# e-sha/dvs_of_training_framework

Hardware: AMD Instinct MI355X
Metric: training samples/sec (256x256x5 event voxels) (higher is better)
Workload: dtype f32; 1 GPU; EV_FlowNet 256x256x5-bin synthetic events, batch 8 per GPU, fp32 (BASELINE.json configs[1]); full step: voxelise + fwd + multi-scale loss + bwd + AdamW-amsgrad; global_batch=8, parallelism=dp1

## Files before the change

dvs_of_training_framework_amd/conv.py:

```python
import ctypes

import torch

from . import _lib

_vp = ctypes.c_void_p
_C = _lib.CONSTANTS

ACT_NONE, ACT_RELU, ACT_MISH = _C['DVSOF_ACT_NONE'], _C['DVSOF_ACT_RELU'], _C['DVSOF_ACT_MISH']
NHWC, NCHW = _C['DVSOF_NHWC'], _C['DVSOF_NCHW']
WGRAD_SKIP_FLAT = _C['DVSOF_CONV_WGRAD_SKIP_FLAT']

Src = _lib.STRUCTS['dvsof_src_t']
ConvDesc = _lib.STRUCTS['dvsof_conv_desc_t']
GradDst = _lib.STRUCTS['dvsof_grad_dst_t']

MFMA_F32, MFMA_BF16, MFMA_BF16X3, MFMA_BF16_TWINS = 0, 1, 2, 3


def twin(t):
    return torch.empty(t.shape, dtype=torch.bfloat16, device=t.device)


def to_bf16(src):
    dst = torch.empty(src.numel(), dtype=torch.bfloat16, device=src.device)
    _lib.check(_lib.lib().dvsof_to_bf16(src.data_ptr(), dst.data_ptr(),
                                         src.numel(), _lib.stream()),
               'dvsof_to_bf16')
    return dst


def to_bf16_many(tensors):
    tensors = list(tensors)
    out = [torch.empty(t.numel(), dtype=torch.bfloat16, device=t.device)
           for t in tensors]
    for i in range(0, len(tensors), 16):
        chunk, dst = tensors[i:i + 16], out[i:i + 16]
        n = len(chunk)
        src_p = (_vp * n)(*[t.data_ptr() for t in chunk])
        dst_p = (_vp * n)(*[t.data_ptr() for t in dst])
        sizes = (ctypes.c_size_t * n)(*[t.numel() for t in chunk])
        _lib.check(_lib.lib().dvsof_to_bf16_many(src_p, dst_p, sizes, n,
                                                  _lib.stream()),
                   'dvsof_to_bf16_many')
    return out


UP_NONE, UP_NEAREST, UP_ZERO = 0, 1, 2

_KERNELS = sorted((v, k[len('DVSOF_KERNEL_'):]) for k, v in _C.items() if k.startswith('DVSOF_KERNEL_'))
assert [v for v, _ in _KERNELS] == list(range(len(_KERNELS)))
globals().update(('K_' + name, v) for v, name in _KERNELS)
KERNEL_NAMES = tuple(name.lower() for _, name in _KERNELS)


def last_kernel(kind):
    v = _lib.lib().dvsof_conv2d_last_kernel(kind)
    return v & 255, v >> 8


def make_desc(srcs, B, H, W, Cout, ksize=3, stride=1, pad=1, upsample=False,
              act=ACT_NONE, mfma=MFMA_F32):
    d = ConvDesc()
    d.nsrc = len(srcs)
    for i, src in enumerate(srcs):
        t, C, layout = src[:3]
        d.src[i].p = t.data_ptr()
        d.src[i].C = C
        d.src[i].layout = layout
        d.src[i].p16 = _lib.ptr(src[3]) if len(src) > 3 else None
    d.B, d.H, d.W = B, H, W
    if upsample is True or upsample is False:
        upsample = UP_NEAREST if upsample else UP_NONE
    assert upsample in (UP_NONE, UP_NEAREST, UP_ZERO)
    d.upsample = upsample
    d.ksize, d.stride, d.pad = ksize, stride, pad
    d.Cout, d.act, d.mfma = Cout, act, mfma
    return d


def out_size(desc):
    up = 2 if desc.upsample else 1
    ho = (desc.H * up + 2 * desc.pad - desc.ksize) // desc.stride + 1
    wo = (desc.W * up + 2 * desc.pad - desc.ksize) // desc.stride + 1
    return ho, wo


_PLAN = {}


def _plan(desc):
    key = (desc.nsrc, tuple((desc.src[i].C, desc.src[i].layout)
                            for i in range(desc.nsrc)), desc.B, desc.H, desc.W,
           desc.upsample, desc.ksize, desc.stride, desc.pad, desc.Cout,
           desc.mfma)
    p = _PLAN.get(key)
    if p is None:
        lib, ref = _lib.lib(), ctypes.byref(desc)
        raw = desc.Cout * desc.ksize ** 2 * sum(desc.src[i].C
                                                for i in range(desc.nsrc))
        p = _PLAN[key] = (raw, lib.dvsof_conv2d_fwd_weight_elems(ref),
                          lib.dvsof_conv2d_dgrad_weight_elems(ref),
                          lib.dvsof_conv2d_scratch_bytes(ref),
                          lib.dvsof_conv2d_wgrad_workspace_bytes(ref))
    return p


def _scratch(desc, device):
    n = _plan(desc)[3]
    if n == 0:
        desc.scratch, desc.scratch_bytes = None, 0
        return None
    t = torch.empty(n // 4, dtype=torch.float32, device=device)
    desc.scratch, desc.scratch_bytes = t.data_ptr(), n
    return t


def winograd_chain(desc, kind):
    return bool(_lib.lib().dvsof_conv2d_winograd_chain(ctypes.byref(desc), kind))


def winograd_tile(desc, kind):
    return _lib.lib().dvsof_conv2d_winograd_tile(ctypes.byref(desc), kind)


def winograd_form(desc, channels, device):
    tiles = desc.B * (desc.H // 4) * (desc.W // 4)
    return torch.empty(36 * tiles * channels, dtype=torch.float32, device=device)


def _chain(desc, pre=None, nxt=None, nxt_gout=None, gout=None):
    desc.winograd_pre = _lib.ptr(pre)
    desc.winograd_next = _lib.ptr(nxt)
    desc.winograd_next_gout = _lib.ptr(nxt_gout)
    desc.winograd_gout = _lib.ptr(gout)


def conv_fwd(desc, weight, bias, device, residual=None, want_z=False,
             keep_input_transform=False, weight16=None, bias_cls=None,
             wino_pre=None, wino_next=None):
    ho, wo = out_size(desc)
    y = torch.empty(desc.B, ho, wo, desc.Cout, dtype=torch.float32,
                    device=device)
    z = torch.empty_like(y) if want_z else None
    desc._y16 = twin(y) if desc.mfma == MFMA_BF16_TWINS else None
    desc.y16 = _lib.ptr(desc._y16)
    desc.w16 = _lib.ptr(weight16)
    desc.bias_cls = _lib.ptr(bias_cls)
    ws = _scratch(desc, device)
    _chain(desc, pre=wino_pre, nxt=wino_next)
    _lib.check(_lib.lib().dvsof_conv2d_fwd(
        ctypes.byref(desc), weight.data_ptr(), _lib.ptr(bias),
        _lib.ptr(residual), y.data_ptr(), _lib.ptr(z), _lib.stream()),
        'dvsof_conv2d_fwd')
    _chain(desc)
    desc._wino_input = (wino_pre if wino_pre is not None else ws) \
        if keep_input_transform else None
    return y, z


def prepare(desc, weight, want_dgrad, phase_weights=None, want16=False):
    lib = _lib.lib()
    raw, nf, ndg, nscratch, _ = _plan(desc)
    dg_only = phase_weights is not None
    if dg_only:
        w_fwd = phase_weights
    else:
        w_fwd = weight if nf == raw else torch.empty(
            nf, dtype=torch.float32, device=weight.device)
    w_dg = torch.empty(ndg, dtype=torch.float32, device=weight.device) \
        if want_dgrad else None
    make_fwd = not dg_only and nf != raw
    w_fwd16 = w_dg16 = None
    if make_fwd or want_dgrad:
        wino = nscratch > 0
        wp = weight.data_ptr()
        fp = w_fwd.data_ptr() if (nf != raw) else None
        if dg_only:
            fp = None
        if want16 and not wino:
            dev = weight.device
            if make_fwd or (nf == raw and want_dgrad and not dg_only):
                w_fwd16 = torch.empty(nf, dtype=torch.bfloat16, device=dev)
            if want_dgrad:
                w_dg16 = torch.empty(ndg, dtype=torch.bfloat16, device=dev)
            _lib.check(lib.dvsof_conv2d_prepare16(
                ctypes.byref(desc), wp, fp, _lib.ptr(w_dg), _lib.ptr(w_fwd16),
                _lib.ptr(w_dg16), _lib.stream()), 'dvsof_conv2d_prepare16')
        else:
            _lib.check(lib.dvsof_conv2d_prepare(
                ctypes.byref(desc), wp, fp, _lib.ptr(w_dg), _lib.stream()),
                'dvsof_conv2d_prepare')
            if want16:
                w_fwd16 = to_bf16(w_fwd) if make_fwd else None
                w_dg16 = to_bf16(w_dg) if w_dg is not None else None
    if want16:
        return w_fwd, w_dg, w_fwd16, w_dg16
    return w_fwd, w_dg


def flip_transpose(weight, Cout, ksize, Ctot):
    wt = torch.empty(Ctot * ksize * ksize * Cout, dtype=torch.float32,
                     device=weight.device)
    _lib.check(_lib.lib().dvsof_weight_flip_transpose(
        weight.data_ptr(), wt.data_ptr(), Cout, ksize, Ctot, _lib.stream()),
        'dvsof_weight_flip_transpose')
    return wt


def conv_dgrad(desc, weight_t, gout, dsts, bwd_act=ACT_NONE, weight16=None,
               gout16=None, wino_pre=None, wino_next=None, wino_next_gout=None):
    arr = (GradDst * len(dsts))()
    for i, d in enumerate(dsts):
        arr[i].p = d['p'].data_ptr()
        arr[i].addend = _lib.ptr(d.get('addend'))
        arr[i].addend2 = _lib.ptr(d.get('addend2'))
        arr[i].actsrc = _lib.ptr(d.get('actsrc'))
        arr[i].p16 = _lib.ptr(d.get('p16'))
        arr[i].head_w = _lib.ptr(d.get('head_w'))
        arr[i].head_gflow = _lib.ptr(d.get('head_gflow'))
        arr[i].head_x = _lib.ptr(d.get('head_x'))
        arr[i].head_part = _lib.ptr(d.get('head_part'))
    desc.w16 = _lib.ptr(weight16)
    desc.gout16 = _lib.ptr(gout16)
    ws = _scratch(desc, gout.device)
    _chain(desc, pre=wino_pre, nxt=wino_next, nxt_gout=wino_next_gout)
    _lib.check(_lib.lib().dvsof_conv2d_dgrad(
        ctypes.byref(desc), weight_t.data_ptr(), gout.data_ptr(), arr,
        bwd_act, _lib.stream()), 'dvsof_conv2d_dgrad')
    _chain(desc)


def flow_fold_weights(w, Cout, Ctot, cx_off, Cx, cf_off, wh):
    out = torch.empty(Cout * 9 * (Ctot - 2), dtype=torch.float32, device=w.device)
    _lib.check(_lib.lib().dvsof_flow_fold_weights(
        w.data_ptr(), Cout, Ctot, cx_off, Cx, cf_off, wh.data_ptr(),
        out.data_ptr(), _lib.stream()), 'dvsof_flow_fold_weights')
    return out


def flow_fold_bias(w, Cout, Ctot, cf_off, bh, bias):
    be = torch.empty(Cout, dtype=torch.float32, device=w.device)
    bc = torch.empty(9 * Cout, dtype=torch.float32, device=w.device)
    _lib.check(_lib.lib().dvsof_flow_fold_bias(
        w.data_ptr(), Cout, Ctot, cf_off, bh.data_ptr(), _lib.ptr(bias),
        be.data_ptr(), bc.data_ptr(), _lib.stream()), 'dvsof_flow_fold_bias')
    return be, bc


def flow_fold_grads(dW, w, Cout, Ctot, cx_off, Cx, cf_off, wh, bh, db_conv, g,
                    B, H, W, dwh, dbh):
    n = _lib.lib().dvsof_flow_fold_workspace_bytes(B, Cout)
    ws = torch.empty(n // 4 + 1, dtype=torch.float32, device=g.device)
    _lib.check(_lib.lib().dvsof_flow_fold_grads(
        dW.data_ptr(), w.data_ptr(), Cout, Ctot, cx_off, Cx, cf_off,
        wh.data_ptr(), bh.data_ptr(), db_conv.data_ptr(), g.data_ptr(), B, H,
        W, dwh.data_ptr(), dbh.data_ptr(), ws.data_ptr(), ws.numel() * 4,
        _lib.stream()), 'dvsof_flow_fold_grads')


def conv_wgrad(desc, gout, dweight, dbias, gout16=None, skip_flat=False,
               wino_gout=None):
    desc.gout16 = _lib.ptr(gout16)
    desc.flags = WGRAD_SKIP_FLAT if skip_flat else 0
    nbytes = _plan(desc)[4]
    ws = torch.empty(max(nbytes // 4, 4), dtype=torch.float32,
                     device=gout.device)
    kept = getattr(desc, '_wino_input', None)
    desc.winograd_input = kept.data_ptr() if kept is not None else None
    _chain(desc, gout=wino_gout)
    _lib.check(_lib.lib().dvsof_conv2d_wgrad(
        ctypes.byref(desc), gout.data_ptr(), dweight.data_ptr(),
        _lib.ptr(dbias), ws.data_ptr(), ws.numel() * 4, _lib.stream()),
        'dvsof_conv2d_wgrad')
    _chain(desc)


def first_dgrad(gz, weight, B, C, H, W):
    _lib.require_cuda(gz, weight)
    assert gz.dtype == torch.float32 and gz.is_contiguous()
    assert gz.numel() == B * (H // 2) * (W // 2) * 64
    assert tuple(weight.shape) == (64, C, 3, 3) and \
        weight.permute(0, 2, 3, 1).is_contiguous(), \
        'enc.0 weight: channels_last [64,C,3,3]'
    out = torch.empty(B, C, H, W, dtype=torch.float32, device=gz.device)
    _lib.check(_lib.lib().dvsof_first_dgrad(
        gz.data_ptr(), weight.data_ptr(), B, C, H, W, out.data_ptr(),
        _lib.stream()), 'dvsof_first_dgrad')
    return out


def head_fwd(x, w, bias, B, H, W, C):
    flow = torch.empty(B, 2, H, W, dtype=torch.float32, device=x.device)
    _lib.check(_lib.lib().dvsof_flow_head_fwd(
        x.data_ptr(), w.data_ptr(), _lib.ptr(bias), flow.data_ptr(), B, H, W,
        C, _lib.stream()), 'dvsof_flow_head_fwd')
    return flow


def heads_fwd(items, B, out=None):
    n = len(items)
    flows = out if out is not None else [
        torch.empty(B, 2, H, W, dtype=torch.float32, device=x.device)
        for x, _, _, H, W, _ in items]
    arr = lambda ts: (_vp * n)(*[_lib.ptr(t) for t in ts])
    ints = lambda k: (ctypes.c_int * n)(*[it[k] for it in items])
    _lib.check(_lib.lib().dvsof_flow_heads_fwd(
        n, arr([it[0] for it in items]), arr([it[1] for it in items]),
        arr([it[2] for it in items]), arr(flows), B, ints(3), ints(4), ints(5),
        _lib.stream()), 'dvsof_flow_heads_fwd')
    return flows


def dgrad_fuses_head(desc):
    return bool(_lib.lib().dvsof_conv2d_dgrad_fuses_head(ctypes.byref(desc)))


def dgrad_head_rows(desc):
    return _lib.lib().dvsof_conv2d_dgrad_head_rows(ctypes.byref(desc))


def dgrad_head_part(desc, C, device):
    rows = _lib.lib().dvsof_conv2d_dgrad_head_rows(ctypes.byref(desc))
    if rows <= 0:
        return None
    return torch.empty(rows, 2 * C + 2, dtype=torch.float32, device=device)


def head_reduce(part, C, dw, dbias):
    _lib.check(_lib.lib().dvsof_flow_head_reduce(
        part.data_ptr(), part.shape[0], C, dw.data_ptr(), _lib.ptr(dbias),
        _lib.stream()), 'dvsof_flow_head_reduce')


def head_bwd(x, w, gflow, gx_in, actsrc, act, gx, dw, dbias, B, H, W, C,
             gx16=None):
    nbytes = _lib.lib().dvsof_flow_head_bwd_workspace_bytes(B, H, W, C)
    ws = torch.empty(nbytes // 4, dtype=torch.float32, device=x.device)
    _lib.check(_lib.lib().dvsof_flow_head_bwd(
        x.data_ptr(), w.data_ptr(), gflow.data_ptr(), _lib.ptr(gx_in),
        _lib.ptr(actsrc), act, _lib.ptr(gx), dw.data_ptr(),
        _lib.ptr(dbias), B, H, W, C, ws.data_ptr(), nbytes, _lib.ptr(gx16),
        _lib.stream()), 'dvsof_flow_head_bwd')


def act_bwd(dy, actsrc, act, out=None):
    out = dy if out is None else out
    _lib.check(_lib.lib().dvsof_act_bwd(
        dy.data_ptr(), actsrc.data_ptr(), act, out.data_ptr(), dy.numel(),
        _lib.stream()), 'dvsof_act_bwd')
    return out
```

dvs_of_training_framework_amd/csrc/conv_api.hip:

```cpp
#include "conv_host.h"

static thread_local int t_last_kernel[3] = {0, 0, 0};
static thread_local int t_kind = 0;
void conv_note_kernel(int family, int mode) { t_last_kernel[t_kind] = family | mode << 8; }
static void conv_begin(int kind)
{
    t_kind = kind;
    t_last_kernel[kind] = DVSOF_KERNEL_NONE;
}
static int conv_retag(int rc, int family)
{
    if (rc == DVSOF_OK && t_last_kernel[t_kind]) conv_note_kernel(family, t_last_kernel[t_kind] >> 8);
    return rc;
}

namespace {

GSrc make_src(const float *p, int C, int layout, int H, int W, const void *p16 = nullptr)
{
    GSrc s;
    s.p = p;
    s.p16 = layout == DVSOF_NHWC ? (const unsigned short *)p16 : nullptr;
    s.C = C;
    if (layout == DVSOF_NCHW) {
        s.sb = (long long)C * H * W;
        s.sy = W;
        s.sx = 1;
        s.sc = H * W;
        s.flat = 1;
    } else {
        s.sb = (long long)H * W * C;
        s.sy = W * C;
        s.sx = C;
        s.sc = 1;
        s.flat = ((C & 3) || C < BK) ? 1 : 0;
    }
    return s;
}

bool desc_ok(const dvsof_conv_desc_t *d, int &Ctot, int &Ho, int &Wo)
{
    if (!d || d->nsrc < 1 || d->nsrc > 3 || d->B < 1 || d->H < 1 || d->W < 1) return false;
    if (d->ksize != 1 && d->ksize != 3 && d->ksize != 5) return false;
    if (d->stride != 1 && d->stride != 2) return false;
    if (d->upsample < 0 || d->upsample > 2) return false;
    if (d->upsample && d->stride != 1) return false;
    if (d->upsample == 2 &&
        !(d->ksize == 3 && d->pad == 1 && d->nsrc == 1 && d->src[0].layout == DVSOF_NHWC &&
          d->src[0].C % BK == 0 && d->mfma != 3))
        return false;
    if (d->Cout < 1 || d->pad < 0 || d->pad >= d->ksize) return false;
    Ctot = 0;
    for (int i = 0; i < d->nsrc; ++i) {
        if (!d->src[i].p || d->src[i].C < 1) return false;
        Ctot += d->src[i].C;
    }
    const int up = d->upsample ? 2 : 1;
    Ho = (d->H * up + 2 * d->pad - d->ksize) / d->stride + 1;
    Wo = (d->W * up + 2 * d->pad - d->ksize) / d->stride + 1;
    if (Ho < 1 || Wo < 1) return false;
    if ((long long)d->B * Ho * Wo > 0x7fffffffLL) return false;
    if ((long long)d->B * d->H * up * d->W * up > 0x7fffffffLL) return false;
    return true;
}

int operand_mode(const dvsof_conv_desc_t *d) { return (d->mfma >= 1 && d->mfma <= 3) ? d->mfma : 0; }

template <class Params>
void layer_geometry(Params &P, const dvsof_conv_desc_t *d, const ConvClass &c)
{
    const int up = d->upsample ? 2 : 1;
    P.B = d->B;
    P.Hv = d->H * up;
    P.Wv = d->W * up;
    P.up = d->upsample ? UP_NEAREST : UP_NONE;
    P.Ho = c.Ho;
    P.Wo = c.Wo;
    P.stride = d->stride;
    P.pad = d->pad;
    P.ks = d->ksize;
    P.M = d->B * c.Ho * c.Wo;
}

template <class Params>
void four_phases(Params &P, int h, int w, int pad, int ph_pad)
{
    P.up = UP_NONE;
    P.Hv = P.Ho = h;
    P.Wv = P.Wo = w;
    P.ks = 2;
    P.stride = 1;
    P.pad = pad;
    P.M = P.B * h * w;
    P.nph = 4;
    P.ph_pad = ph_pad;
}
void phase_strides(int &sy, int &sx, int &ph_y, int &ph_x)
{
    ph_y = sy;
    ph_x = sx;
    sy *= 2;
    sx *= 2;
}

void fill_wgrad(const dvsof_conv_desc_t *d, const ConvClass &c, WGradParams &P)
{
    P.mfma_bf16 = d->mfma == 3 ? 1 : operand_mode(d);
    P.nsrc = d->nsrc;
    for (int i = 0; i < d->nsrc; ++i)
        P.src[i] = make_src(d->src[i].p, d->src[i].C, d->src[i].layout, d->H, d->W,
                            d->mfma == 3 ? d->src[i].p16 : nullptr);
    P.gout16 = d->mfma == 3 ? (const unsigned short *)d->gout16 : nullptr;
    P.twins = P.gout16 != nullptr && (d->Cout % 8) == 0;
    for (int i = 0; i < d->nsrc; ++i)
        if (!P.src[i].flat && (!P.src[i].p16 || (P.src[i].C % 8))) P.twins = 0;
    layer_geometry(P, d, c);
    P.Cout = d->Cout;
    P.Cin_tot = c.Ctot;
    P.nph = 1;
    P.S = 1;
    P.g_sb = (long long)c.Ho * c.Wo * d->Cout;
    P.g_sy = c.Wo * d->Cout;
    P.g_sx = d->Cout;
    if (c.wgrad == WG_SUBPIXEL) {
        four_phases(P, d->H, d->W, d->pad, 1);
        phase_strides(P.g_sy, P.g_sx, P.g_py, P.g_px);
    }
}

int fill_flat(const dvsof_conv_desc_t *d, const ConvClass &c, const float *gout, FlatWG *F)
{
    int n = 0, coff = 0;
    for (int i = 0; i < d->nsrc; ++i) {
        const GSrc g = make_src(d->src[i].p, d->src[i].C, d->src[i].layout, d->H, d->W);
        if (g.flat) {
            FlatWG &f = F[n++];
            f.S = g;
            f.gout = gout;
            layer_geometry(f, d, c);
            f.Cout = d->Cout;
            f.ncol = d->ksize * d->ksize * g.C;
            f.coff = coff;
            f.Cin_tot = c.Ctot;
        }
        coff += d->src[i].C;
    }
    return n;
}

__global__ __launch_bounds__(256) void channel_sum_partial_kernel(const float *__restrict__ g,
                                                                  long long npix, int C,
                                                                  float *__restrict__ part)
{
    const int per = 256 / C, c = threadIdx.x % C, r = threadIdx.x / C;
    float a = 0.f;
    if (r < per)
        for (long long p = (long long)blockIdx.x * per + r; p < npix; p += (long long)gridDim.x * per)
            a += g[p * C + c];
    __shared__ float sm[256];
    sm[threadIdx.x] = a;
    __syncthreads();
    if (threadIdx.x < C) {
        float t = 0.f;
        for (int j = 0; j < per; ++j) t += sm[j * C + threadIdx.x];
        part[(size_t)blockIdx.x * C + threadIdx.x] = t;
    }
}
__global__ __launch_bounds__(256) void channel_sum_final_kernel(const float *__restrict__ part,
                                                                int nblocks, int C,
                                                                float *__restrict__ out)
{
    const int c = blockIdx.x * 4 + (threadIdx.x >> 6), lane = threadIdx.x & 63;
    if (c >= C) return;
    double a = 0;
    for (int b = lane; b < nblocks; b += 64) a += (double)part[(size_t)b * C + c];
    a = wave_sum(a);
    if (lane == 0) out[c] = (float)a;
}

}

ConvClass conv_classify(const dvsof_conv_desc_t *d)
{
    ConvClass c = {};
    c.ok = desc_ok(d, c.Ctot, c.Ho, c.Wo);
    if (!c.ok) return c;
    const bool subpixel = d->upsample == 1 && d->ksize == 3 && d->pad == 1 && d->stride == 1;
    const bool transposed = d->upsample == 2;
    const bool phased2 = !d->upsample && d->stride == 2 && d->ksize == 3 && d->pad == 1 &&
                         (d->H % 2 == 0) && (d->W % 2 == 0);
    const bool first = first_layer_shape(d->nsrc, d->src[0].layout == DVSOF_NCHW, d->src[0].C, d->Cout, d->H,
                                         d->W, d->ksize, d->stride, d->pad, d->upsample) && !d->bias_cls;
    const bool wino = d->nsrc == 1 &&
                      wino_eligible_shape(d->nsrc, d->src[0].layout == DVSOF_NHWC, d->src[0].C, d->Cout, d->B,
                                          d->H, d->W, d->ksize, d->stride, d->pad, d->upsample, d->mfma);
    c.wino_mode = d->mfma == 2 ? 2 : 0;
    const int wg_tile = wino ? wino_wgrad_tile(d->B, d->H, d->W, c.wino_mode) : 0;
    bool min9 = false, min9_dgrad = false;
    if (subpixel) {
        int C[3] = {0, 0, 0}, nhwc[3] = {0, 0, 0};
        for (int i = 0; i < d->nsrc; ++i) {
            C[i] = d->src[i].C;
            nhwc[i] = d->src[i].layout == DVSOF_NHWC;
        }
        min9 = min9_shape_ok(d->mfma, d->nsrc, C, nhwc, d->Cout, d->H, d->W);
        min9_dgrad = min9 && min9_dgrad_shape_ok(C, d->Cout, d->H);
    }
    c.fwd = first ? FWD_FIRST : wino ? FWD_WINO : min9 ? FWD_MIN9 : subpixel ? FWD_SUBPIXEL
          : transposed ? FWD_TRANSPOSED : FWD_GENERAL;
    c.dgrad = min9_dgrad ? DG_MIN9 : wino ? DG_WINO : subpixel ? DG_SUBPIXEL : phased2 ? DG_PHASED2
            : transposed ? DG_TRANSPOSED : d->upsample ? DG_QUAD : d->stride == 2 ? DG_ZERO2 : DG_PLAIN;
    c.wgrad = transposed ? WG_TRANSPOSED : wg_tile ? WG_WINO : first ? WG_FIRST : subpixel ? WG_SUBPIXEL
            : WG_GENERAL;
    if (wino) {
        c.wino_tile[0] = c.wino_tile[1] = wino_tile(d->B, d->H, d->W, c.wino_mode);
        c.wino_tile[2] = wg_tile;
        c.wino_chain[0] = wino_chain_ok(d->B, d->H, d->W, d->Cout, c.wino_mode);
        c.wino_chain[1] = wino_chain_ok(d->B, d->H, d->W, c.Ctot, c.wino_mode);
    }
    c.head_folds = min9_dgrad || (subpixel && d->src[0].layout == DVSOF_NHWC);
    return c;
}

extern "C" {

int dvsof_conv2d_fwd(const dvsof_conv_desc_t *d, const float *weight, const float *bias,
                     const float *residual, float *y, float *z, void *stream)
{
    conv_begin(0);
    const ConvClass c = conv_classify(d);
    if (!c.ok || !weight || !y) return DVSOF_EINVAL;
    hipStream_t st = as_stream(stream);
    unsigned short *y16 = d->mfma == 3 ? (unsigned short *)d->y16 : nullptr;
    if (c.fwd == FWD_FIRST && !residual)
        return first_fwd_launch(d->src[0].p, d->B, c.Ctot, d->H, d->W, weight, bias, d->act, y, z, y16, st);
    if (d->winograd_next_gout || (c.fwd != FWD_WINO && (d->winograd_pre || d->winograd_next)))
        return DVSOF_EINVAL;
    const int Cout = d->Cout;
    GConvParams P = {};
    P.nsrc = d->nsrc;
    for (int i = 0; i < d->nsrc; ++i)
        P.src[i] = make_src(d->src[i].p, d->src[i].C, d->src[i].layout, d->H, d->W, d->src[i].p16);
    P.ndst = 1;
    P.dst[0] = {y, residual, nullptr, nullptr, (long long)c.Ho * c.Wo * Cout, c.Wo * Cout, Cout, 1, Cout, 0, 0, y16};
    P.W = weight;
    P.W16 = d->mfma == 3 ? (const unsigned short *)d->w16 : nullptr;
    P.bias = bias;
    P.bias_cls = d->bias_cls;
    P.out_H = c.Ho;
    P.out_W = c.Wo;
    P.zout = z;
    layer_geometry(P, d, c);
    P.N = Cout;
    P.Cin_tot = c.Ctot;
    P.act = d->act;
    P.mfma_bf16 = operand_mode(d);
    P.bwd_act = ACT_NONE;
    P.nph = 1;
    switch (c.fwd) {
    case FWD_WINO: {
        const WinoChain ch = {d->winograd_pre, d->winograd_next, nullptr};
        return wino_launch(P, (float *)d->scratch, d->scratch_bytes / sizeof(float), ch, st);
    }
    case FWD_MIN9:
    case FWD_SUBPIXEL:
        four_phases(P, d->H, d->W, d->pad, 1);
        break;
    case FWD_TRANSPOSED:
        four_phases(P, d->H, d->W, 0, 0);
        P.ph_exact = 1;
        break;
    default: break;
    }
    if (P.nph == 4) {
        P.w_phase_stride = (long long)Cout * 4 * c.Ctot;
        phase_strides(P.dst[0].sy, P.dst[0].sx, P.dst[0].ph_y, P.dst[0].ph_x);
    }
    if (c.fwd == FWD_MIN9) return fwd_min_launch(P, st);
    if (c.fwd == FWD_SUBPIXEL && fwd_patch_eligible(P))
        return fwd_patch_launch(P, st);
    const int rc = gconv_launch(P, 0, st);
    return c.fwd == FWD_TRANSPOSED ? conv_retag(rc, DVSOF_KERNEL_TRANSPOSED) : rc;
}

int dvsof_conv2d_dgrad_fuses_head(const dvsof_conv_desc_t *d)
{
    const ConvClass c = conv_classify(d);
    return c.ok && c.head_folds ? 1 : 0;
}

int dvsof_conv2d_dgrad_head_rows(const dvsof_conv_desc_t *d)
{
    const ConvClass c = conv_classify(d);
    if (!c.ok || c.dgrad != DG_MIN9) return 0;
    return d->B * (d->H / 8) * (d->W / 16);
}

int dvsof_conv2d_dgrad(const dvsof_conv_desc_t *d, const float *weight_t, const float *gout,
                       const dvsof_grad_dst_t *dst, int bwd_act, void *stream)
{
    conv_begin(1);
    const ConvClass c = conv_classify(d);
    if (!c.ok || !weight_t || !gout || !dst) return DVSOF_EINVAL;
    hipStream_t st = as_stream(stream);
    GConvParams P = {};
    P.nsrc = 1;
    P.src[0] = make_src(gout, d->Cout, DVSOF_NHWC, c.Ho, c.Wo, d->mfma == 3 ? d->gout16 : nullptr);
    P.ndst = d->nsrc;
    for (int i = 0; i < d->nsrc; ++i) {
        if (!dst[i].p) return DVSOF_EINVAL;
        const GSrc g = make_src(nullptr, d->src[i].C, d->src[i].layout, d->H, d->W);
        P.dst[i] = {dst[i].p, dst[i].addend, dst[i].addend2, dst[i].actsrc, g.sb, g.sy, g.sx, g.sc, g.C, 0, 0,
                    (d->mfma == 3 && d->src[i].layout == DVSOF_NHWC) ? (unsigned short *)dst[i].p16 : nullptr,
                    dst[i].head_w, dst[i].head_gflow, dst[i].head_x, dst[i].head_part};
        if ((dst[i].head_w != nullptr) != (dst[i].head_gflow != nullptr)) return DVSOF_EINVAL;
        if ((dst[i].head_x != nullptr) != (dst[i].head_part != nullptr)) return DVSOF_EINVAL;
        if (dst[i].head_part && (!dst[i].head_w || i != 0)) return DVSOF_EINVAL;
        if (dst[i].head_w && (i != 0 || !c.head_folds)) return DVSOF_EINVAL;
        if (dst[i].head_part && c.dgrad != DG_MIN9) return DVSOF_EINVAL;
    }
    P.W = weight_t;
    P.W16 = d->mfma == 3 ? (const unsigned short *)d->w16 : nullptr;
    P.B = d->B;
    P.N = c.Ctot;
    P.Cin_tot = d->Cout;
    P.act = ACT_NONE;
    P.mfma_bf16 = operand_mode(d);
    P.bwd_act = bwd_act;
    P.nph = 1;
    P.up = UP_NONE;
    P.Hv = c.Ho;
    P.Wv = c.Wo;
    P.Ho = d->H;
    P.Wo = d->W;
    P.ks = d->ksize;
    P.stride = 1;
    P.pad = d->ksize - 1 - d->pad;
    switch (c.dgrad) {
    case DG_MIN9:
    case DG_SUBPIXEL:
        P.ks = 4;
        P.stride = 2;
        P.pad = 1;
        break;
    case DG_PHASED2:
        four_phases(P, d->H / 2, d->W / 2, 0, 0);
        P.ph_exact = 1;
        P.w_phase_stride = (long long)c.Ctot * 4 * d->Cout;
        for (int i = 0; i < d->nsrc; ++i) phase_strides(P.dst[i].sy, P.dst[i].sx, P.dst[i].ph_y, P.dst[i].ph_x);
        break;
    case DG_TRANSPOSED:
        P.stride = 2;
        P.pad = 1;
        break;
    case DG_QUAD:
        P.Ho = 2 * d->H;
        P.Wo = 2 * d->W;
        P.quad = 1;
        break;
    case DG_ZERO2:
        P.up = UP_ZERO;
        P.Hv = 2 * c.Ho;
        P.Wv = 2 * c.Wo;
        break;
    default: break;
    }
    P.M = d->B * P.Ho * P.Wo;
    if (c.dgrad == DG_MIN9) return dgrad_min_launch(P, st);
    if (c.dgrad == DG_WINO) {
        const WinoChain ch = {d->winograd_pre, d->winograd_next, d->winograd_next_gout};
        return wino_launch(P, (float *)d->scratch, d->scratch_bytes / sizeof(float), ch, st);
    }
    if (d->winograd_pre || d->winograd_next || d->winograd_next_gout) return DVSOF_EINVAL;
    const int rc = gconv_launch(P, 0, st);
    return c.dgrad == DG_PHASED2 ? conv_retag(rc, DVSOF_KERNEL_STRIDE2_PHASED) : rc;
}

size_t dvsof_conv2d_scratch_bytes(const dvsof_conv_desc_t *d)
{
    const ConvClass c = conv_classify(d);
    if (!c.ok || c.fwd != FWD_WINO) return 0;
    return wino_scratch_floats(d->B, d->H, d->W, c.Ctot, d->Cout, c.wino_mode) * sizeof(float);
}

static dvsof_conv_desc_t adjoint_of_transposed(const dvsof_conv_desc_t *d, int Ctot, const float *gy)
{
    dvsof_conv_desc_t a = *d;
    a.nsrc = 1;
    a.src[0].p = gy;
    a.src[0].C = d->Cout;
    a.src[0].layout = DVSOF_NHWC;
    a.src[0].p16 = nullptr;
    a.H = 2 * d->H;
    a.W = 2 * d->W;
    a.upsample = 0;
    a.stride = 2;
    a.Cout = Ctot;
    a.scratch = nullptr;
    a.scratch_bytes = 0;
    a.winograd_input = nullptr;
    return a;
}
static int channel_sum_blocks(long long npix, int C)
{
    const long long per = 256 / C, want = (npix + per * 8 - 1) / (per * 8);
    return (int)(want < 1 ? 1 : want > 1024 ? 1024 : want);
}

size_t dvsof_conv2d_wgrad_workspace_bytes(const dvsof_conv_desc_t *d)
{
    const ConvClass c = conv_classify(d);
    if (!c.ok) return 0;
    switch (c.wgrad) {
    case WG_TRANSPOSED: {
        static const float dummy = 0.f;
        const dvsof_conv_desc_t a = adjoint_of_transposed(d, c.Ctot, &dummy);
        size_t n = dvsof_conv2d_wgrad_workspace_bytes(&a);
        n = (n + 255) & ~(size_t)255;
        n += (size_t)c.Ctot * 9 * d->Cout * sizeof(float);
        if (d->Cout <= 256)
            n += (size_t)channel_sum_blocks((long long)d->B * c.Ho * c.Wo, d->Cout) * d->Cout * sizeof(float);
        return n + 256;
    }
    case WG_WINO:
        return wino_wgrad_workspace_floats(d->B, d->H, d->W, c.Ctot, d->Cout, c.wino_mode) * sizeof(float) + 16;
    default: break;
    }
    WGradParams P = {};
    fill_wgrad(d, c, P);
    FlatWG F[3] = {};
    const int nflat = fill_flat(d, c, nullptr, F);
    size_t n = wgrad_plan(P, F, nflat, true, true).total;
    if (c.wgrad == WG_FIRST) {
        const size_t nf = first_wgrad_workspace_floats(d->B, c.Ctot, d->H, d->W);
        if (nf > n) n = nf;
    }
    return n * sizeof(float) + 16;
}

int dvsof_conv2d_wgrad(const dvsof_conv_desc_t *d, const float *gout, float *dweight, float *dbias,
                       void *ws, size_t ws_bytes, void *stream)
{
    conv_begin(2);
    const ConvClass c = conv_classify(d);
    if (!c.ok || !gout || !dweight) return DVSOF_EINVAL;
    hipStream_t st = as_stream(stream);
    const bool skip_flat = (d->flags & DVSOF_CONV_WGRAD_SKIP_FLAT) != 0;
    switch (c.wgrad) {
    case WG_TRANSPOSED: {
        if (dbias && d->Cout > 256) return DVSOF_EINVAL;
        const dvsof_conv_desc_t a = adjoint_of_transposed(d, c.Ctot, gout);
        size_t wsa = dvsof_conv2d_wgrad_workspace_bytes(&a);
        wsa = (wsa + 255) & ~(size_t)255;
        const size_t need = dvsof_conv2d_wgrad_workspace_bytes(d);
        if (!ws || ws_bytes < need) return DVSOF_ENOSPACE;
        float *dw_adj = (float *)((char *)ws + wsa);
        float *part = dw_adj + (size_t)c.Ctot * 9 * d->Cout;
        int rc = dvsof_conv2d_wgrad(&a, d->src[0].p, dw_adj, nullptr, ws, wsa, stream);
        if (rc) return rc;
        rc = dvsof_weight_flip_transpose(dw_adj, dweight, c.Ctot, 3, d->Cout, stream);
        if (rc) return rc;
        if (dbias) {
            const long long npix = (long long)d->B * c.Ho * c.Wo;
            const int nb = channel_sum_blocks(npix, d->Cout);
            hipLaunchKernelGGL(channel_sum_partial_kernel, dim3(nb), dim3(256), 0, st, gout, npix, d->Cout, part);
            DVSOF_LAUNCH_CHECK();
            hipLaunchKernelGGL(channel_sum_final_kernel, dim3((d->Cout + 3) / 4), dim3(256), 0, st,
                               (const float *)part, nb, d->Cout, dbias);
            DVSOF_LAUNCH_CHECK();
        }
        return DVSOF_OK;
    }
    case WG_WINO: {
        const float *v_in = c.wino_tile[0] == c.wino_tile[2] ? d->winograd_input : nullptr;
        const float *z_in = c.wino_tile[2] == 4 ? d->winograd_gout : nullptr;
        return wino_wgrad_launch(make_src(d->src[0].p, d->src[0].C, d->src[0].layout, d->H, d->W), v_in, z_in,
                                 gout, dweight, dbias, d->B, d->H, d->W, c.Ctot, d->Cout, c.wino_mode, (float *)ws,
                                 ws_bytes / sizeof(float), st);
    }
    case WG_FIRST:
        if (!skip_flat)
            return first_wgrad_launch(d->src[0].p, d->B, c.Ctot, d->H, d->W, gout, dweight, dbias, (float *)ws,
                                      ws_bytes / sizeof(float), st);
        break;
    default: break;
    }
    WGradParams P = {};
    fill_wgrad(d, c, P);
    P.gout = gout;
    FlatWG F[3] = {};
    const int nflat = skip_flat ? 0 : fill_flat(d, c, gout, F);
    return wgrad_launch(P, dweight, dbias, (float *)ws, ws_bytes / sizeof(float), F, nflat, st);
}

size_t dvsof_conv2d_fwd_weight_elems(const dvsof_conv_desc_t *d)
{
    const ConvClass c = conv_classify(d);
    if (!c.ok) return 0;
    const bool phases = c.fwd == FWD_MIN9 || c.fwd == FWD_SUBPIXEL || c.fwd == FWD_TRANSPOSED;
    return (size_t)d->Cout * c.Ctot * (c.fwd == FWD_WINO ? wino_components(d->B, d->H, d->W, c.wino_mode)
                                       : phases ? 16 : d->ksize * d->ksize);
}

size_t dvsof_conv2d_dgrad_weight_elems(const dvsof_conv_desc_t *d)
{
    const ConvClass c = conv_classify(d);
    if (!c.ok) return 0;
    const bool taps16 = c.dgrad == DG_MIN9 || c.dgrad == DG_SUBPIXEL || c.dgrad == DG_PHASED2;
    return (size_t)d->Cout * c.Ctot * (c.dgrad == DG_WINO ? wino_components(d->B, d->H, d->W, c.wino_mode)
                                       : taps16 ? 16 : d->ksize * d->ksize);
}

int dvsof_conv2d_winograd_tile(const dvsof_conv_desc_t *d, int kind)
{
    const ConvClass c = conv_classify(d);
    return c.ok ? c.wino_tile[kind == 2 ? 2 : 0] : 0;
}

int dvsof_conv2d_winograd_chain(const dvsof_conv_desc_t *d, int kind)
{
    const ConvClass c = conv_classify(d);
    return c.ok && (kind == 0 || kind == 1) && c.wino_chain[kind] ? 1 : 0;
}

int dvsof_conv2d_kernel_generation(const dvsof_conv_desc_t *d, int kind)
{
    const ConvClass c = conv_classify(d);
    if (!c.ok) return DVSOF_EINVAL;
    if (kind != 1 && c.fwd == FWD_FIRST) return 3;
    if (kind == 2) {
        for (int i = 0; i < d->nsrc; ++i) {
            const GSrc g = make_src(d->src[i].p, d->src[i].C, d->src[i].layout, d->H, d->W);
            if (!g.flat) return (c.Wo % BK == 0 && (!d->upsample || c.wgrad == WG_SUBPIXEL)) ? 2 : 1;
        }
        return 0;
    }
    if (kind == 1) return (d->Cout % BK == 0) ? 2 : 1;
    for (int i = 0; i < d->nsrc; ++i) {
        const GSrc g = make_src(d->src[i].p, d->src[i].C, d->src[i].layout, d->H, d->W);
        if (!g.flat) return (g.C % BK == 0) ? 2 : 1;
    }
    return 1;
}

int dvsof_conv2d_last_kernel(int kind)
{
    return (kind >= 0 && kind <= 2) ? t_last_kernel[kind] : 0;
}

int dvsof_conv2d_last_patch(int kind)
{
    switch (dvsof_conv2d_last_kernel(kind) & 255) {
    case DVSOF_KERNEL_FWD_MIN4:
    case DVSOF_KERNEL_FWD_MIN8:
    case DVSOF_KERNEL_DGRAD_MIN0:
    case DVSOF_KERNEL_DGRAD_MIN1:
    case DVSOF_KERNEL_DGRAD_MIN2:
    case DVSOF_KERNEL_WGRAD_MIN: return 2;
    case DVSOF_KERNEL_FWD_PATCH:
    case DVSOF_KERNEL_WGRAD_PATCH: return 1;
    default: return 0;
    }
}

int dvsof_conv2d_tile_id(const dvsof_conv_desc_t *d, int kind)
{
    const ConvClass c = conv_classify(d);
    if (!c.ok) return DVSOF_EINVAL;
    if (kind == 0) return gconv_pick_tile((long long)d->B * c.Ho * c.Wo, d->Cout);
    if (kind == 1) {
        const int up = (c.dgrad == DG_QUAD || c.dgrad == DG_TRANSPOSED) ? 2 : 1;
        int n = c.Ctot, trail = 0;
        for (int i = d->nsrc - 1; i > 0; --i) {
            const GSrc g = make_src(d->src[i].p, d->src[i].C, d->src[i].layout, d->H, d->W);
            if (!g.flat || trail + g.C > 4) break;
            trail += g.C;
        }
        if (up == 1 && c.dgrad != DG_PHASED2 && n - trail >= 32) n -= trail;
        return gconv_pick_tile((long long)d->B * d->H * up * d->W * up, n);
    }
    if (kind == 2) {
        WGradParams P = {};
        fill_wgrad(d, c, P);
        return wgrad_plan(P, nullptr, 0, false, true).tile;
    }
    return DVSOF_EINVAL;
}

}
```

dvs_of_training_framework_amd/csrc/conv_common.h:

```cpp
#pragma once
#include "common.h"

typedef float f32x16 __attribute__((ext_vector_type(16)));
typedef float f32x4 __attribute__((ext_vector_type(4)));
typedef float f32x4u __attribute__((ext_vector_type(4), aligned(4)));
typedef float f32x8 __attribute__((ext_vector_type(8)));
typedef __bf16 bf16x8 __attribute__((ext_vector_type(8)));

enum { UP_NONE = 0, UP_NEAREST = 1, UP_ZERO = 2 };
enum { ACT_NONE = 0, ACT_RELU = 1, ACT_MISH = 2 };

constexpr int CONV_NT = 256;
constexpr int BK = 16;
constexpr int LDK = BK + 4;

struct GSrc {
    const float *p;
    long long sb;
    int sy, sx, sc;
    int C;
    int flat;
    const unsigned short *p16;
};

struct GDst {
    float *p;
    const float *addend;
    const float *addend2;
    const float *actsrc;
    long long sb;
    int sy, sx, sc;
    int C;
    int ph_y, ph_x;
    unsigned short *p16;
    const float *head_w;
    const float *head_g;
    const float *head_x;
    float *head_part;
};

struct GConvParams {
    GSrc src[3];
    GDst dst[3];
    const float *W;
    const unsigned short *W16;
    const float *bias;
    const float *bias_cls;
    int out_H, out_W;
    float *zout;
    int nsrc, ndst;
    int B, Hv, Wv;
    int up;
    int Ho, Wo;
    int stride, pad, ks;
    int nph;
    int ph_pad;
    long long w_phase_stride;
    long long src_ph_stride;
    int N, Cin_tot, M;
    int quad;
    int act;
    int bwd_act;
    int mfma_bf16;
    int ph_exact;
    int xcd;
    int dbg;
};

struct WinoChain {
    const float *v_pre;
    float *v_next;
    float *z_next;
};

struct WGradParams {
    GSrc src[3];
    const float *gout;
    float *dW;
    float *dbias;
    int nsrc;
    int B, Hv, Wv, up, Ho, Wo, stride, pad, ks;
    int Cout, Cin_tot, M;
    int klen;
    int tile_begin[4];
    long long g_sb;
    int g_sy, g_sx;
    int g_py, g_px;
    int nph, ph_pad, S;
    int mfma_bf16;
    long long src_ph_stride;
    const unsigned short *gout16;
    int twins;
    int xcd;
};

struct FlatWG {
    GSrc S;
    const float *gout;
    int B, Hv, Wv, up, Ho, Wo, stride, pad, ks, Cout, M, ncol;
    int coff, Cin_tot;
};

__device__ __forceinline__ float mish_t(float x, float &n)
{
    n = __builtin_amdgcn_exp2f(fminf(x, 20.f) * 1.4426950408889634f);
    return n * (n + 2.f);
}

__device__ __forceinline__ unsigned short bf16_bits(float v)
{
    const __bf16 h = (__bf16)v;
    return __builtin_bit_cast(unsigned short, h);
}

__device__ __forceinline__ float act_fwd(float v, int act)
{
    if (act == ACT_RELU) return fmaxf(v, 0.f);
    if (act == ACT_MISH) {
        float n;
        const float t = mish_t(v, n);
        return v * (t * __builtin_amdgcn_rcpf(t + 2.f));
    }
    return v;
}

__device__ __forceinline__ float act_bwd(float s, int act)
{
    if (act == ACT_RELU) return s > 0.f ? 1.f : 0.f;
    if (act == ACT_MISH) {
        float n;
        const float t = mish_t(s, n);
        const float r = __builtin_amdgcn_rcpf(t + 2.f);
        const float th = t * r;
        const float sg = n * __builtin_amdgcn_rcpf(1.f + n);
        return th + (s > 20.f ? 20.f : s) * ((2.f * r) * (1.f + th)) * sg;
    }
    return 1.f;
}

template <int MODE, int TM, int TN>
__device__ __forceinline__ void mfma_k16(f32x16 (&acc)[TM][TN], const f32x4 (&a)[2][TM],
                                         const f32x4 (&b)[2][TN])
{
    if constexpr (MODE == 0) {
#pragma unroll
        for (int j = 0; j < 2; ++j)
#pragma unroll
            for (int i = 0; i < 4; ++i)
#pragma unroll
                for (int tm = 0; tm < TM; ++tm)
#pragma unroll
                    for (int tn = 0; tn < TN; ++tn)
                        acc[tm][tn] = __builtin_amdgcn_mfma_f32_32x32x2f32(a[j][tm][i], b[j][tn][i],
                                                                           acc[tm][tn], 0, 0, 0);
    } else {
        bf16x8 ah[TM], bh[TN], al[TM], bl[TN];
#pragma unroll
        for (int t = 0; t < TM; ++t) {
            const f32x8 v = __builtin_shufflevector(a[0][t], a[1][t], 0, 1, 2, 3, 4, 5, 6, 7);
            ah[t] = __builtin_convertvector(v, bf16x8);
            if constexpr (MODE == 2)
                al[t] = __builtin_convertvector(v - __builtin_convertvector(ah[t], f32x8), bf16x8);
        }
#pragma unroll
        for (int t = 0; t < TN; ++t) {
            const f32x8 v = __builtin_shufflevector(b[0][t], b[1][t], 0, 1, 2, 3, 4, 5, 6, 7);
            bh[t] = __builtin_convertvector(v, bf16x8);
            if constexpr (MODE == 2)
                bl[t] = __builtin_convertvector(v - __builtin_convertvector(bh[t], f32x8), bf16x8);
        }
#pragma unroll
        for (int tm = 0; tm < TM; ++tm)
#pragma unroll
            for (int tn = 0; tn < TN; ++tn) {
                if constexpr (MODE == 2) {
                    acc[tm][tn] = __builtin_amdgcn_mfma_f32_32x32x16_bf16(al[tm], bh[tn], acc[tm][tn], 0, 0, 0);
                    acc[tm][tn] = __builtin_amdgcn_mfma_f32_32x32x16_bf16(ah[tm], bl[tn], acc[tm][tn], 0, 0, 0);
                }
                acc[tm][tn] = __builtin_amdgcn_mfma_f32_32x32x16_bf16(ah[tm], bh[tn], acc[tm][tn], 0, 0, 0);
            }
    }
}

__device__ __forceinline__ void conv_row_offsets(const GConvParams &P, long long *rowO, int *rowC, int BM,
                                                 int r, bool valid, int b, int oy, int ox, int phy,
                                                 int phx)
{
    if (P.bias_cls) {
        const int Y = P.nph == 4 ? 2 * oy + phy : oy, X = P.nph == 4 ? 2 * ox + phx : ox;
        rowC[r] = valid ? 3 * (Y == 0 ? 1 : Y == P.out_H - 1 ? 2 : 0) + (X == 0 ? 1 : X == P.out_W - 1 ? 2 : 0)
                        : 0;
    }
    if (P.dst[0].head_w) rowC[r] = valid ? (b * 2 * P.Ho + oy) * P.Wo + ox : -1;
    if (P.quad) {
        oy >>= 1;
        ox >>= 1;
    }
    for (int d = 0; d < P.ndst; ++d) {
        const GDst &D = P.dst[d];
        rowO[d * BM + r] = valid ? (long long)b * D.sb + (long long)oy * D.sy + (long long)ox * D.sx +
                                       (long long)phy * D.ph_y + (long long)phx * D.ph_x
                                 : -1;
    }
}

template <int TM, int TN>
__device__ __forceinline__ void conv_epilogue(const GConvParams &P, f32x16 (&acc)[TM][TN],
                                              const long long *rowO, const int *rowC, int BM, int n0,
                                              int wr, int wc, int lane)
{
    const int lrow = lane & 31;
    bool has_add = false, has_add2 = false, has_as = false;
    for (int d = 0; d < P.ndst; ++d) {
        has_add |= P.dst[d].addend != nullptr;
        has_add2 |= P.dst[d].addend2 != nullptr;
        has_as |= P.dst[d].actsrc != nullptr;
    }
#pragma unroll
    for (int tn = 0; tn < TN; ++tn) {
        const int n = n0 + (wc * TN + tn) * 32 + lrow;
        const bool col_ok = n < P.N;
        int dsel = 0, off = 0, run = 0;
        float *dp = P.dst[0].p;
        unsigned short *dp16 = P.dst[0].p16;
        const float *a1 = P.dst[0].addend, *a2 = P.dst[0].addend2, *as = P.dst[0].actsrc;
        int sc = P.dst[0].sc;
        for (int d = 1; d < P.ndst; ++d) {
            run += P.dst[d - 1].C;
            if (n >= run) {
                dsel = d;
                off = run;
                dp = P.dst[d].p;
                dp16 = P.dst[d].p16;
                a1 = P.dst[d].addend;
                a2 = P.dst[d].addend2;
                as = P.dst[d].actsrc;
                sc = P.dst[d].sc;
            }
        }
        const long long *ro = rowO + dsel * BM;
        const long long cpart = (long long)(n - off) * sc;
        const float bias = (P.bias && col_ok) ? P.bias[n] : 0.f;
#ifdef DVSOF_NO_GENERAL_HEAD
        const bool has_head = false;
#else
        const bool has_head = P.dst[0].head_w != nullptr;
#endif
        float hw0 = 0.f, hw1 = 0.f;
        if (has_head && dsel == 0 && col_ok) {
            hw0 = P.dst[0].head_w[n];
            hw1 = P.dst[0].head_w[P.dst[0].C + n];
        }
#pragma unroll
        for (int tm = 0; tm < TM; ++tm) {
            const int rbase = (wr * TM + tm) * 32 + 4 * (lane >> 5);
            if (!P.quad) {
                long long o[16];
                float v[16];
#pragma unroll
                for (int reg = 0; reg < 16; ++reg) {
                    const long long r_ = ro[rbase + (reg & 3) + 8 * (reg >> 2)];
                    o[reg] = (col_ok && r_ >= 0) ? r_ + cpart : -1;
                    v[reg] = acc[tm][tn][reg] + bias;
                }
                if (P.bias_cls) {
#pragma unroll
                    for (int reg = 0; reg < 16; ++reg) {
                        const int c = rowC[rbase + (reg & 3) + 8 * (reg >> 2)];
                        if (c != 0 && col_ok) v[reg] += P.bias_cls[c * P.N + n];
                    }
                }
                if (has_add) {
                    float t[16];
#pragma unroll
                    for (int reg = 0; reg < 16; ++reg) t[reg] = (a1 && o[reg] >= 0) ? a1[o[reg]] : 0.f;
#pragma unroll
                    for (int reg = 0; reg < 16; ++reg) v[reg] = a1 ? v[reg] + t[reg] : v[reg];
                }
                if (has_add2) {
                    float t[16];
#pragma unroll
                    for (int reg = 0; reg < 16; ++reg) t[reg] = (a2 && o[reg] >= 0) ? a2[o[reg]] : 0.f;
#pragma unroll
                    for (int reg = 0; reg < 16; ++reg) v[reg] = a2 ? v[reg] + t[reg] : v[reg];
                }
                if (has_head) {
                    const long long hwp = (long long)P.Ho * P.Wo;
                    float g0[16], g1[16];
#pragma unroll
                    for (int reg = 0; reg < 16; ++reg) {
                        const int rg = rowC[rbase + (reg & 3) + 8 * (reg >> 2)];
                        g0[reg] = rg >= 0 ? P.dst[0].head_g[rg] : 0.f;
                        g1[reg] = rg >= 0 ? P.dst[0].head_g[rg + hwp] : 0.f;
                    }
#pragma unroll
                    for (int reg = 0; reg < 16; ++reg) v[reg] += g0[reg] * hw0 + g1[reg] * hw1;
                }
                if (has_as) {
                    float t[16];
#pragma unroll
                    for (int reg = 0; reg < 16; ++reg) t[reg] = (as && o[reg] >= 0) ? as[o[reg]] : 0.f;
#pragma unroll
                    for (int reg = 0; reg < 16; ++reg)
                        v[reg] = as ? v[reg] * act_bwd(t[reg], P.bwd_act) : v[reg];
                }
                if (P.zout) {
#pragma unroll
                    for (int reg = 0; reg < 16; ++reg)
                        if (o[reg] >= 0) P.zout[o[reg]] = v[reg];
                }
#pragma unroll
                for (int reg = 0; reg < 16; ++reg) v[reg] = act_fwd(v[reg], P.act);
#pragma unroll
                for (int reg = 0; reg < 16; ++reg)
                    if (o[reg] >= 0) dp[o[reg]] = v[reg];
                if (dp16) {
#pragma unroll
                    for (int reg = 0; reg < 16; ++reg)
                        if (o[reg] >= 0) dp16[o[reg]] = bf16_bits(v[reg]);
                }
            } else {
                long long o[4];
                float v[4];
#pragma unroll
                for (int g = 0; g < 4; ++g) {
                    const long long r_ = ro[rbase + 8 * g];
                    o[g] = (col_ok && r_ >= 0) ? r_ + cpart : -1;
                    v[g] = (acc[tm][tn][4 * g] + acc[tm][tn][4 * g + 1]) +
                           (acc[tm][tn][4 * g + 2] + acc[tm][tn][4 * g + 3]) + bias;
                }
                float t1[4], t2[4], t3[4];
#pragma unroll
                for (int g = 0; g < 4; ++g) {
                    t1[g] = (a1 && o[g] >= 0) ? a1[o[g]] : 0.f;
                    t2[g] = (a2 && o[g] >= 0) ? a2[o[g]] : 0.f;
                    t3[g] = (as && o[g] >= 0) ? as[o[g]] : 0.f;
                }
#pragma unroll
                for (int g = 0; g < 4; ++g) {
                    if (a1) v[g] += t1[g];
                    if (a2) v[g] += t2[g];
                    if (as) v[g] *= act_bwd(t3[g], P.bwd_act);
                    if (o[g] >= 0) dp[o[g]] = v[g];
                    if (dp16 && o[g] >= 0) dp16[o[g]] = bf16_bits(v[g]);
                }
            }
        }
    }
}
```

dvs_of_training_framework_amd/csrc/conv_host.h:

```cpp
#pragma once
#include "conv_common.h"

enum ConvFwdForm { FWD_GENERAL, FWD_FIRST, FWD_WINO, FWD_MIN9, FWD_SUBPIXEL, FWD_TRANSPOSED };
enum ConvDgradForm { DG_PLAIN, DG_MIN9, DG_WINO, DG_SUBPIXEL, DG_PHASED2, DG_TRANSPOSED, DG_QUAD, DG_ZERO2 };
enum ConvWgradForm { WG_GENERAL, WG_TRANSPOSED, WG_WINO, WG_FIRST, WG_SUBPIXEL };

struct ConvClass {
    bool ok;
    int Ctot, Ho, Wo;
    ConvFwdForm fwd;
    ConvDgradForm dgrad;
    ConvWgradForm wgrad;
    int wino_mode;
    int wino_tile[3];
    bool wino_chain[2];
    bool head_folds;
};
ConvClass conv_classify(const dvsof_conv_desc_t *d);

void conv_note_kernel(int family, int mode);

int gconv_launch(const GConvParams &P, int tile_hint, hipStream_t st);
int gconv_pick_tile(long long m, long long n);
bool gconv2_eligible(const GConvParams &P, long long max_src_bytes, long long w_bytes);
int gconv2_launch(const GConvParams &P, int tile, hipStream_t st);

enum WGVec { WGV_NONE, WGV_V1, WGV_V2, WGV_PATCH_TWINS, WGV_PATCH_F32, WGV_MIN9 };
enum WGFlat { WGF_NONE, WGF_V1, WGF_OWN };
enum WGBias { WGB_NONE, WGB_VECTOR, WGB_COLSUM, WGB_FLAT };
enum WGReduce { WGR_NONE, WGR_SLABS, WGR_SUBPIXEL, WGR_PATCH };
constexpr int WG_COLSUM_BLOCKS = 512;
constexpr int WG_FLAT_BLOCKS = 512;
constexpr int WG_MIN_CT = 64;
struct WGradPlan {
    int rc;
    WGVec vec;
    int tile, bn;
    int ntiles;
    int S, klen;
    WGFlat flat;
    bool flat_mfma[3];
    WGBias bias;
    bool bias_tail;
    WGReduce reduce;
    int zg;
    size_t bias_off, flat_off[3], total;
    int family, mode;
};
WGradPlan wgrad_plan(const WGradParams &P, const FlatWG *flat, int nflat, bool with_bias, bool sizing);
int wgrad_enumerate_tiles(WGradParams &P, int cols_per_channel, int width, bool vec, bool flat);
bool wgrad2_eligible(const WGradParams &P);
int wgrad_launch(WGradParams P, float *dW, float *dbias, float *ws, size_t ws_floats,
                 const FlatWG *flat, int nflat, hipStream_t st);
int wgrad2_launch(const WGradParams &P, int tile, int ntiles, hipStream_t st);
int wgrad_patch_launch(const WGradParams &P, bool f32, int ct, hipStream_t st);
int wgrad_min_launch(const WGradParams &P, hipStream_t st);
template <void (*KERNEL)(const WGradParams), int CT, int NT, int LDS>
int wgrad_resident_launch(const WGradParams &P0, hipStream_t st)
{
    WGradParams P = P0;
    const int nt = wgrad_enumerate_tiles(P, 1, CT, true, false);
    static bool attr_set = false;
    if (!attr_set) {
        DVSOF_HIP_TRY(hipFuncSetAttribute((const void *)KERNEL, hipFuncAttributeMaxDynamicSharedMemorySize, LDS));
        attr_set = true;
    }
    P.xcd = 1;
    hipLaunchKernelGGL(KERNEL, dim3(nt, P.Cout / 32, P.S), dim3(NT), LDS, st, P);
    DVSOF_LAUNCH_CHECK();
    return DVSOF_OK;
}

bool wino_eligible_shape(int nsrc, int layout_nhwc, int C, int N, int B, int H, int W, int ksize,
                         int stride, int pad, int upsample, int mfma);
int wino_tile(int B, int H, int W, int mfma);
int wino_components(int B, int H, int W, int mfma);
bool wino_chain_ok(int B, int H, int W, int N, int mfma);
size_t wino_scratch_floats(int B, int H, int W, int C, int N, int mfma);
int wino_prepare(const float *weight, float *U, float *Ut, int N, int C, int B, int H, int W, int mfma,
                 hipStream_t st);
int wino_launch(const GConvParams &P, float *scratch, size_t scratch_floats, const WinoChain &ch, hipStream_t st);
int wino_wgrad_tile(int B, int H, int W, int mfma);
size_t wino_wgrad_workspace_floats(int B, int H, int W, int C, int N, int mfma);
int wino_wgrad_launch(const GSrc &X, const float *V_in, const float *Z_in, const float *gout, float *dW, float *dbias, int B,
                      int H, int W, int C, int N, int mfma_bf16, float *ws, size_t ws_floats,
                      hipStream_t st);

bool first_layer_shape(int nsrc, int planar, int C, int Cout, int H, int W, int ksize, int stride,
                       int pad, int upsample);
int first_fwd_launch(const float *x, int B, int C, int H, int W, const float *w, const float *bias,
                     int act, float *y, float *z, unsigned short *y16, hipStream_t st);
size_t first_wgrad_workspace_floats(int B, int C, int H, int W);
int first_wgrad_launch(const float *x, int B, int C, int H, int W, const float *gout, float *dW,
                       float *dbias, float *ws, size_t ws_floats, hipStream_t st);

bool fwd_patch_eligible(const GConvParams &P);
int fwd_patch_launch(const GConvParams &P, hipStream_t st);
bool min9_shape_ok(int mfma, int nsrc, const int *C, const int *nhwc, int Cout, int H, int W);
int min9_prepare_fwd(const float *w, float *wt, int Cout, int Ctot, hipStream_t st);
int fwd_min_launch(const GConvParams &P, hipStream_t st);
bool min9_dgrad_shape_ok(const int *C, int Cout, int H);
int min9_prepare_dgrad(const float *w, float *wq, int Cout, int Ctot, hipStream_t st);
int dgrad_min_launch(const GConvParams &P, hipStream_t st);
```

dvs_of_training_framework_amd/csrc/dgrad_min.hip:

```cpp
#include "conv_host.h"
#include <stdlib.h>

namespace {

constexpr unsigned DM_OOB = 0x80000000u;
constexpr int DM_NT = 512;
constexpr int DM_NR = 8;
constexpr int DM_AARR = 9 * 1024 + 16;
constexpr int DM_AP = 4 * 9;
constexpr int DM_PR = 17;
constexpr int DM_NPAIR = (2 * DM_NR + 2) * DM_PR;
constexpr int DM_BPA = 5;
constexpr int DM_BARR = DM_BPA * 1024 + 16;
constexpr int DM_BOFF = 4 * DM_AARR;
constexpr int DM_BP = 8 * DM_BPA;
constexpr int DM_NPIECE = DM_AP + DM_BP;
constexpr int DM_LPW = (DM_NPIECE + 7) / 8;
constexpr int DM_STAGE = ((DM_BOFF + 8 * DM_BARR + 1023) / 1024) * 1024;
constexpr int DM_LDS = 2 * DM_STAGE;

__global__ __launch_bounds__(256) void min9_dgrad_weights_kernel(const float *__restrict__ w, float *__restrict__ wq,
                                                                 int Cout, int Ctot)
{
    __shared__ float tile[32][33];
    const int z = blockIdx.z, p = z / 3, q = z - 3 * p;
    const int ci0 = blockIdx.x * 32, co0 = blockIdx.y * 32;
    const int lx = threadIdx.x & 31, ly = threadIdx.x >> 5;
    for (int r = ly; r < 32; r += 8) {
        const int co = co0 + r, ci = ci0 + lx;
        float v = 0.f;
        if (co < Cout && ci < Ctot) {
            const float *k = w + (size_t)co * 9 * Ctot + ci;
            auto col = [&](int kx) -> float {
                const float *kc = k + (size_t)kx * Ctot;
                return p == 0 ? kc[3 * Ctot] + kc[6 * Ctot] : p == 1 ? kc[0] : kc[6 * Ctot];
            };
            v = q == 0 ? col(1) + col(2) : q == 1 ? col(0) : col(2);
        }
        tile[r][lx] = v;
    }
    __syncthreads();
    for (int r = ly; r < 32; r += 8) {
        const int ci = ci0 + r, co = co0 + lx;
        if (ci < Ctot && co < Cout) wq[((size_t)z * Ctot + ci) * Cout + co] = tile[lx][r];
    }
}

template <int IPW>
__global__ __launch_bounds__(DM_NT) void dgrad_min_f32_kernel(const GConvParams P, const int total)
{
#if defined(__HIP_DEVICE_COMPILE__)
    typedef float f32x2 __attribute__((ext_vector_type(2)));
    extern __shared__ __attribute__((aligned(1024))) unsigned char smem[];
    const int tid = threadIdx.x, lane = tid & 63;
    const int wave = __builtin_amdgcn_readfirstlane(tid >> 6);
    const int pt = wave & 3, ks = wave >> 2;
    const int lrow = lane & 31, lh = lane >> 5;
    const int H = P.Ho, W = P.Wo;
    const int FH = 2 * H, FW = 2 * W;
    const int Cout = P.Cin_tot, Ctot = P.N;
    const int nbx = W / 16, nby = H / DM_NR;
    const int nct = Ctot / 64;
    const int nchunks = Cout / 16;

    unsigned wg = blockIdx.x;
    {
        const unsigned tot = gridDim.x, x = wg & 7u, q = tot >> 3, r = tot & 7u;
        wg = x * q + min(x, r) + (wg >> 3);
    }
    constexpr bool RES = IPW == 0;
    const int rows = RES ? (int)gridDim.x / nct : 1;
    const int item0 = RES ? ((int)wg / nct) * nct + (int)wg % nct : (int)wg * IPW;
    const int istep = RES ? rows * nct : 1;
    const int item1 = RES ? total : item0 + IPW;

    const GSrc &GS = P.src[0];
    const __amdgpu_buffer_rsrc_t wres = __builtin_amdgcn_make_buffer_rsrc((void *)P.W, 0, 0x7fffffff, 0x00020000);
    const __amdgpu_buffer_rsrc_t gres = __builtin_amdgcn_make_buffer_rsrc(
        (void *)(GS.p - ((long long)GS.sy + GS.sx)), 0, 0x7fffffff, 0x00020000);

    unsigned off[DM_LPW];
    int ci0 = 0, b = 0, oy = 0, ox = 0, wbase = 0, gbase = 0, blk_ = 0;
    auto setup = [&](int item) {
        const int ct64 = item % nct, blk = item / nct;
        blk_ = blk;
        ci0 = 64 * ct64;
        const int bx = blk % nbx, by = (blk / nbx) % nby;
        b = blk / (nbx * nby);
        oy = DM_NR * by;
        ox = 16 * bx;
        wbase = __builtin_amdgcn_readfirstlane((int)((size_t)ci0 * Cout * 4));
        gbase = __builtin_amdgcn_readfirstlane(
            (int)(((long long)b * GS.sb + (long long)(2 * oy) * GS.sy + (long long)(2 * ox) * GS.sx) * 4));
#pragma unroll
        for (int i = 0; i < DM_LPW; ++i) {
            const int p = wave + 8 * i;
            if (p < DM_AP) {
                const int m = p / 9, pp = p - 9 * m;
                const int j = 16 * pp + (lane >> 2);
                const int c = j >> 4, r = 4 * (j & 15) + m;
                off[i] = (unsigned)((((size_t)c * Ctot + r) * Cout + 4 * (lane & 3)) * 4);
            } else if (p < DM_NPIECE) {
                off[i] = DM_OOB;
                const int pb = p - DM_AP;
                const int arr = pb / DM_BPA, pp = pb - DM_BPA * arr;
                const int pr = 4 * (16 * pp + (lane >> 2)) + (arr & 3);
                if (pr < DM_NPAIR) {
                    const int n = 2 * pr + (arr >> 2);
                    const int fr = n / 34, fc = n - 34 * fr;
                    if (((unsigned)(2 * oy + fr - 1) < (unsigned)FH) & ((unsigned)(2 * ox + fc - 1) < (unsigned)FW))
                        off[i] = (unsigned)((fr * GS.sy + fc * GS.sx + 4 * (lane & 3)) * 4);
                }
            } else {
                off[i] = DM_OOB;
            }
        }
    };

    bool with_w = true;
    auto issue = [&](int stage_idx, int ch) {
        unsigned char *st = smem + stage_idx * DM_STAGE;
        const int so_w = __builtin_amdgcn_readfirstlane(wbase + ch * 64);
        const int so_g = __builtin_amdgcn_readfirstlane(gbase + ch * 64);
#pragma unroll
        for (int i = 0; i < DM_LPW; ++i) {
            const int p = wave + 8 * i;
            if (p < DM_AP) {
                if (RES && !with_w) continue;
                const int m = p / 9, pp = p - 9 * m;
                __attribute__((address_space(3))) void *dst =
                    (__attribute__((address_space(3))) void *)(st + m * DM_AARR + pp * 1024);
                __builtin_amdgcn_raw_ptr_buffer_load_lds(wres, dst, 16, off[i], so_w, 0, 0);
            } else if (p < DM_NPIECE) {
                const int pb = p - DM_AP;
                const int arr = pb / DM_BPA, pp = pb - DM_BPA * arr;
                __attribute__((address_space(3))) void *dst =
                    (__attribute__((address_space(3))) void *)(st + DM_BOFF + arr * DM_BARR + pp * 1024);
                __builtin_amdgcn_raw_ptr_buffer_load_lds(gres, dst, 16, off[i], so_g, 0, 0);
            }
        }
    };

    const int abase = (lrow & 3) * DM_AARR + (lrow >> 2) * 64 + 16 * lh;
    int bb[4][2];
    {
        const int li = lrow >> 4, lj = lrow & 15;
#pragma unroll
        for (int u = 0; u < 4; ++u)
#pragma unroll
            for (int h = 0; h < 2; ++h) {
                const int pr = (2 * (2 * pt + li) + u) * DM_PR + lj + h;
                bb[u][h] = DM_BOFF + (pr & 3) * DM_BARR + (pr >> 2) * 64 + 16 * lh;
            }
    }

    f32x16 acc[2];

    typedef float f32x4_ __attribute__((ext_vector_type(4)));
    auto compute = [&](int u_) {
        const unsigned char *st = smem + u_ * DM_STAGE;
        const int ko = 32 * ks;
        f32x4_ g[4][4];
#pragma unroll
        for (int u = 0; u < 4; ++u)
#pragma unroll
            for (int v = 0; v < 4; ++v)
                g[u][v] = *(const f32x4_ *)(st + bb[u][v >> 1] + (v & 1) * (4 * DM_BARR) + ko);
        f32x4_ cc[4][3], s[9];
#pragma unroll
        for (int u = 0; u < 4; ++u) {
            cc[u][0] = g[u][1] + g[u][2];
            cc[u][1] = g[u][2] + g[u][3];
            cc[u][2] = g[u][0] - g[u][2];
        }
#pragma unroll
        for (int q = 0; q < 3; ++q) {
            s[q] = cc[1][q] + cc[2][q];
            s[3 + q] = cc[2][q] + cc[3][q];
            s[6 + q] = cc[0][q] - cc[2][q];
        }
#pragma unroll
        for (int t = 0; t < 2; ++t)
#pragma unroll
            for (int c = 0; c < 9; ++c) {
                const f32x4_ a = *(const f32x4_ *)(st + abase + (16 * c + 8 * t) * 64 + ko);
#pragma unroll
                for (int j = 0; j < 4; ++j)
                    acc[t] = __builtin_amdgcn_mfma_f32_32x32x2f32(a[j], s[c][j], acc[t], 0, 0, 0);
            }
    };

    if (item0 >= item1) return;
    setup(item0);
    issue(0, 0);
#pragma unroll
    for (int item = item0; item < item1; item += istep) {
        const int e_ci0 = ci0, e_b = b, e_oy = oy, e_ox = ox, e_blk = blk_;
#pragma unroll
        for (int t = 0; t < 2; ++t)
#pragma unroll
            for (int r = 0; r < 16; ++r) acc[t][r] = 0.f;
        for (int ch = 0; ch < nchunks; ++ch) {
            asm volatile("s_waitcnt vmcnt(0)" ::: "memory");
            __builtin_amdgcn_s_barrier();
            if (ch + 1 < nchunks) issue((ch + 1) & 1, ch + 1);
            else if (item + istep < item1) {
                with_w = false;
                setup(item + istep);
                issue((ch + 1) & 1, 0);
            }
            compute(ch & 1);
        }

        unsigned char *xch = RES ? smem + DM_STAGE + DM_BOFF : smem + ((nchunks - 1) & 1) * DM_STAGE;
        const int cit = e_ci0 + 32 * ks;
        const int c_first = P.dst[0].C;
        const int sel = cit >= c_first ? 1 : 0;
        const GDst &D = P.dst[sel];
        const int cm = cit - (sel ? c_first : 0);
        int le = lane;
        asm volatile("" : "+v"(le));
        const int ecq = le & 7, elrow = le & 31, elh = le >> 5;
        f32x4 hw0 = {0.f, 0.f, 0.f, 0.f}, hw1 = hw0;
        if (D.head_w) {
            hw0 = *(const f32x4 *)(D.head_w + cm + 4 * ecq);
            hw1 = *(const f32x4 *)(D.head_w + D.C + cm + 4 * ecq);
        }
        long long eo[4];
        f32x4 ead[4], ead2[4], eas[4], ehx[4];
        float eg0[4], eg1[4];
        const bool hx_own = D.head_part && D.head_x != D.actsrc;
#pragma unroll
        for (int it = 0; it < 4; ++it) {
            const int px = 8 * it + (le >> 3);
            const int yy = e_oy + 2 * pt + (px >> 4), xx = e_ox + (px & 15);
            eo[it] = (long long)e_b * D.sb + (long long)yy * D.sy + (long long)xx * D.sx + cm + 4 * ecq;
            if (D.addend) ead[it] = *(const f32x4 *)(D.addend + eo[it]);
            if (D.addend2) ead2[it] = *(const f32x4 *)(D.addend2 + eo[it]);
            if (D.actsrc) eas[it] = *(const f32x4 *)(D.actsrc + eo[it]);
            if (hx_own) ehx[it] = *(const f32x4 *)(D.head_x + eo[it]);
            if (D.head_w) {
                const long long hwp = (long long)H * W, r = (long long)yy * W + xx;
                eg0[it] = D.head_g[((long long)e_b * 2) * hwp + r];
                eg1[it] = D.head_g[((long long)e_b * 2 + 1) * hwp + r];
            }
        }
        __builtin_amdgcn_s_barrier();
        f32x16 mine = ks ? acc[1] : acc[0];
        {
            const f32x16 other = ks ? acc[0] : acc[1];
            unsigned char *r1 = xch + wave * 4096;
#pragma unroll
            for (int g = 0; g < 4; ++g)
                *(f32x4 *)(r1 + (g * 64 + le) * 16) = f32x4{other[4 * g], other[4 * g + 1], other[4 * g + 2], other[4 * g + 3]};
        }
        __builtin_amdgcn_s_barrier();
        {
            const unsigned char *p1 = xch + (pt + 4 * (1 - ks)) * 4096;
#pragma unroll
            for (int g = 0; g < 4; ++g) {
                const f32x4 o_ = *(const f32x4 *)(p1 + (g * 64 + le) * 16);
#pragma unroll
                for (int e = 0; e < 4; ++e) mine[4 * g + e] = ks ? o_[e] + mine[4 * g + e] : mine[4 * g + e] + o_[e];
            }
        }
        __builtin_amdgcn_s_barrier();
        unsigned char *r2 = xch + wave * 4096;
#pragma unroll
        for (int g = 0; g < 4; ++g) {
            const f32x4 v = {mine[4 * g], mine[4 * g + 1], mine[4 * g + 2], mine[4 * g + 3]};
            *(f32x4 *)(r2 + elrow * 128 + (((2 * g + elh) ^ (elrow & 7)) << 4)) = v;
        }
        f32x4 ha0 = {0.f, 0.f, 0.f, 0.f}, ha1 = ha0;
        float hs0 = 0.f, hs1 = 0.f;
#pragma unroll
        for (int it = 0; it < 4; ++it) {
            const int px = 8 * it + (le >> 3);
            const int xo = px * 128 + ((ecq ^ (px & 7)) << 4);
            f32x4 v = *(const f32x4 *)(r2 + xo);
            if (D.addend) v += ead[it];
            if (D.addend2) v += ead2[it];
            if (D.head_w) v += eg0[it] * hw0 + eg1[it] * hw1;
            if (D.head_part) {
                const f32x4 xv = hx_own ? ehx[it] : eas[it];
                ha0 += eg0[it] * xv;
                ha1 += eg1[it] * xv;
                hs0 += eg0[it];
                hs1 += eg1[it];
            }
            if (D.actsrc) {
#pragma unroll
                for (int e = 0; e < 4; ++e) v[e] *= act_bwd(eas[it][e], P.bwd_act);
            }
            *(f32x4 *)(D.p + eo[it]) = v;
        }
        if (D.head_part) {
#pragma unroll
            for (int o_ = 8; o_ < 64; o_ <<= 1) {
#pragma unroll
                for (int e = 0; e < 4; ++e) {
                    ha0[e] += __shfl_xor(ha0[e], o_, 64);
                    ha1[e] += __shfl_xor(ha1[e], o_, 64);
                }
                hs0 += __shfl_xor(hs0, o_, 64);
                hs1 += __shfl_xor(hs1, o_, 64);
            }
            float *red = (float *)(xch + 32768);
            if (le < 8) {
                *(f32x4 *)(red + (wave * 2 + 0) * 32 + 4 * ecq) = ha0;
                *(f32x4 *)(red + (wave * 2 + 1) * 32 + 4 * ecq) = ha1;
                if (le == 0) {
                    red[512 + wave * 2] = hs0;
                    red[512 + wave * 2 + 1] = hs1;
                }
            }
            __builtin_amdgcn_s_barrier();
            const int Cm = D.C;
            float *prow = D.head_part + (size_t)e_blk * (2 * Cm + 2);
            if (tid < 128) {
                const int ks_ = tid >> 6, k_ = (tid >> 5) & 1, c_ = tid & 31;
                float t_ = 0.f;
#pragma unroll
                for (int p_ = 0; p_ < 4; ++p_) t_ += red[((p_ + 4 * ks_) * 2 + k_) * 32 + c_];
                prow[k_ * Cm + e_ci0 + 32 * ks_ + c_] = t_;
            } else if (tid < 130 && e_ci0 == 0) {
                const int k_ = tid - 128;
                prow[2 * Cm + k_] = (red[512 + 0 + k_] + red[512 + 2 + k_]) + (red[512 + 4 + k_] + red[512 + 6 + k_]);
            }
        }
    }
#endif
}

}

bool min9_dgrad_shape_ok(const int *C, int Cout, int H)
{
    return (C[0] & 63) == 0 && (C[1] & 63) == 0 && (H % DM_NR) == 0 && (Cout & 15) == 0;
}

int min9_prepare_dgrad(const float *w, float *wq, int Cout, int Ctot, hipStream_t st)
{
    dim3 grid((Ctot + 31) / 32, (Cout + 31) / 32, 9);
    hipLaunchKernelGGL(min9_dgrad_weights_kernel, grid, dim3(256), 0, st, w, wq, Cout, Ctot);
    DVSOF_LAUNCH_CHECK();
    return DVSOF_OK;
}

int dgrad_min_launch(const GConvParams &P, hipStream_t st)
{
    const GSrc &S = P.src[0];
    if (!S.p || (reinterpret_cast<uintptr_t>(S.p) & 15) || ((S.sb | S.sy | S.sx) & 3) || S.sc != 1) return DVSOF_EINVAL;
    if (P.ndst != 2 || (reinterpret_cast<uintptr_t>(P.W) & 15)) return DVSOF_EINVAL;
    for (int i = 0; i < 2; ++i) {
        const GDst &D = P.dst[i];
        if (!D.p || D.sc != 1 || ((D.sb | D.sy | D.sx) & 3)) return DVSOF_EINVAL;
        if ((reinterpret_cast<uintptr_t>(D.p) | reinterpret_cast<uintptr_t>(D.addend) |
             reinterpret_cast<uintptr_t>(D.addend2) | reinterpret_cast<uintptr_t>(D.actsrc) |
             reinterpret_cast<uintptr_t>(D.head_w)) & 15)
            return DVSOF_EINVAL;
    }
    static bool attr_set = false;
    if (!attr_set) {
        DVSOF_HIP_TRY(hipFuncSetAttribute((const void *)dgrad_min_f32_kernel<1>,
                                          hipFuncAttributeMaxDynamicSharedMemorySize, DM_LDS));
        attr_set = true;
    }
    const long long total = (long long)P.B * (P.Ho / DM_NR) * (P.Wo / 16) * (P.N / 64);
    const int nchunks = P.Cin_tot / 16;
    const int nct = P.N / 64;
    if (nchunks == 2 && 256 % nct == 0 && total >= 2 * 256) {
        static bool attr0 = false;
        if (!attr0) {
            DVSOF_HIP_TRY(hipFuncSetAttribute((const void *)dgrad_min_f32_kernel<0>,
                                              hipFuncAttributeMaxDynamicSharedMemorySize, DM_LDS));
            attr0 = true;
        }
        hipLaunchKernelGGL(dgrad_min_f32_kernel<0>, dim3(256), dim3(DM_NT), DM_LDS, st, P, (int)total);
        DVSOF_LAUNCH_CHECK();
        conv_note_kernel(DVSOF_KERNEL_DGRAD_MIN0, 0);
        return DVSOF_OK;
    }
    hipLaunchKernelGGL(dgrad_min_f32_kernel<1>, dim3((unsigned)total), dim3(DM_NT), DM_LDS, st, P, (int)total);
    DVSOF_LAUNCH_CHECK();
    conv_note_kernel(DVSOF_KERNEL_DGRAD_MIN1, 0);
    return DVSOF_OK;
}
```

dvs_of_training_framework_amd/csrc/fwd_min.hip:

```cpp
#include "conv_host.h"
#include <stdlib.h>

namespace {

constexpr unsigned FM_OOB = 0x80000000u;
constexpr int FM_NT = 512;
constexpr int FM_APA = 5;
constexpr int FM_AP = 8 * FM_APA;
constexpr int FM_AARR = FM_APA * 1024 + 16;

template <int NR>
struct FMGeom {
    static constexpr int PT = NR / 2;
    static constexpr int KS = 8 / PT;
    static constexpr int SLOTS = (NR + 2) * 18;
    static constexpr int BROWS = (SLOTS + 7) / 8;
    static constexpr int BPA = (BROWS + 7) / 8;
    static constexpr int BARR = BPA * 1024 + 16;
    static constexpr int BOFF = 8 * FM_AARR;
    static constexpr int NPIECE = FM_AP + 8 * BPA;
    static constexpr int LPW = NPIECE / 8;
    static constexpr int STAGE = ((8 * FM_AARR + 8 * BARR + 1023) / 1024) * 1024;
    static constexpr int XCH = 8 * 4 * 4096;
    static constexpr int LDS = 2 * STAGE > XCH ? 2 * STAGE : XCH;
};

__global__ __launch_bounds__(256) void min9_fwd_weights_kernel(const float *__restrict__ w, float *__restrict__ wt,
                                                               int Cout, int Ctot)
{
    const size_t i = (size_t)blockIdx.x * 256 + threadIdx.x;
    if (i >= (size_t)Cout * Ctot) return;
    const int ci = (int)(i % Ctot), co = (int)(i / Ctot);
    float k[3][3], r[3][3];
#pragma unroll
    for (int t = 0; t < 9; ++t) k[t / 3][t % 3] = w[((size_t)co * 9 + t) * Ctot + ci];
#pragma unroll
    for (int l = 0; l < 3; ++l) {
        r[0][l] = k[0][l];
        r[1][l] = (k[0][l] + k[1][l]) + k[2][l];
        r[2][l] = k[2][l];
    }
#pragma unroll
    for (int p = 0; p < 3; ++p) {
        const float v[3] = {r[p][0], (r[p][0] + r[p][1]) + r[p][2], r[p][2]};
#pragma unroll
        for (int q = 0; q < 3; ++q) wt[((size_t)(3 * p + q) * Cout + co) * Ctot + ci] = v[q];
    }
}

template <int NR, bool ZOUT>
__global__ __launch_bounds__(FM_NT) void fwd_min_f32_kernel(const GConvParams P)
{
#if defined(__HIP_DEVICE_COMPILE__)
    typedef FMGeom<NR> G;
    typedef float f32x2 __attribute__((ext_vector_type(2)));
    extern __shared__ __attribute__((aligned(1024))) unsigned char smem[];
    const int tid = threadIdx.x, lane = tid & 63;
    const int wave = __builtin_amdgcn_readfirstlane(tid >> 6);
    const int pt = wave % G::PT, ks = wave / G::PT;
    const int lrow = lane & 31, lh = lane >> 5;
    const int H = P.Hv, W = P.Wv;
    const int nbx = W / 16, nby = H / NR;

    unsigned wg = blockIdx.x;
    {
        const unsigned total = gridDim.x, x = wg & 7u, q = total >> 3, r = total & 7u;
        wg = x * q + min(x, r) + (wg >> 3);
    }
    const int nco = P.N / 32;
    const int cot = (int)(wg % (unsigned)nco), blk = (int)(wg / (unsigned)nco);
    const int co0 = 32 * cot;
    const int bx = blk % nbx, by = (blk / nbx) % nby, b = blk / (nbx * nby);
    const int oy = NR * by, ox = 16 * bx;

    const GSrc &S0 = P.src[0], &S1 = P.src[1];
    unsigned off_a[G::LPW], off_b[G::LPW - FM_APA];
#pragma unroll
    for (int i = 0; i < G::LPW; ++i) {
        const int p = wave + 8 * i;
        off_a[i] = FM_OOB;
        if (i >= FM_APA) off_b[i - FM_APA] = FM_OOB;
        if (i < FM_APA) {
            const int m = p / FM_APA, pp = p - FM_APA * m;
            const int j = 8 * pp + (lane >> 3);
            if (j < 36) {
                const int R = 8 * j + m;
                const int c = R >> 5, r = R & 31;
                off_a[i] = (unsigned)((((size_t)c * P.N + co0 + r) * P.Cin_tot + 4 * (lane & 7)) * 4);
            }
        } else {
            const int pb = p - FM_AP;
            const int m = pb / G::BPA, pp = pb - G::BPA * m;
            const int n = 8 * (8 * pp + (lane >> 3)) + m;
            if (n < G::SLOTS) {
                const int r = n / 18, c = n - 18 * r;
                if (((unsigned)(oy + r - 1) < (unsigned)H) & ((unsigned)(ox + c - 1) < (unsigned)W)) {
                    off_a[i] = (unsigned)((r * S0.sy + c * S0.sx + 4 * (lane & 7)) * 4);
                    off_b[i - FM_APA] = (unsigned)((r * S1.sy + c * S1.sx + 4 * (lane & 7)) * 4);
                }
            }
        }
    }
    const __amdgpu_buffer_rsrc_t wres = __builtin_amdgcn_make_buffer_rsrc((void *)P.W, 0, 0x7fffffff, 0x00020000);
    const __amdgpu_buffer_rsrc_t res0 = __builtin_amdgcn_make_buffer_rsrc(
        (void *)(S0.p - ((long long)S0.sy + S0.sx)), 0, 0x7fffffff, 0x00020000);
    const __amdgpu_buffer_rsrc_t res1 = __builtin_amdgcn_make_buffer_rsrc(
        (void *)(S1.p - ((long long)S1.sy + S1.sx)), 0, 0x7fffffff, 0x00020000);
    const int base0 = __builtin_amdgcn_readfirstlane(
        (int)(((long long)b * S0.sb + (long long)oy * S0.sy + (long long)ox * S0.sx) * 4));
    const int base1 = __builtin_amdgcn_readfirstlane(
        (int)(((long long)b * S1.sb + (long long)oy * S1.sy + (long long)ox * S1.sx) * 4));
    const int nch0 = S0.C / 32, nchunks = P.Cin_tot / 32;

    auto issue = [&](int stage_idx, int ch) {
        unsigned char *st = smem + stage_idx * G::STAGE;
        const bool m1 = ch >= nch0;
        const int so_w = ch * 128;
        const int so_x = m1 ? base1 + (ch - nch0) * 128 : base0 + ch * 128;
#pragma unroll
        for (int i = 0; i < G::LPW; ++i) {
            const int p = wave + 8 * i;
            if (i < FM_APA) {
                const int m = p / FM_APA, pp = p - FM_APA * m;
                __attribute__((address_space(3))) void *dst =
                    (__attribute__((address_space(3))) void *)(st + m * FM_AARR + pp * 1024);
                __builtin_amdgcn_raw_ptr_buffer_load_lds(wres, dst, 16, off_a[i], so_w, 0, 0);
            } else {
                const int pb = p - FM_AP;
                const int m = pb / G::BPA, pp = pb - G::BPA * m;
                __attribute__((address_space(3))) void *dst =
                    (__attribute__((address_space(3))) void *)(st + G::BOFF + m * G::BARR + pp * 1024);
                if (m1)
                    __builtin_amdgcn_raw_ptr_buffer_load_lds(res1, dst, 16, off_b[i - FM_APA], so_x, 0, 0);
                else
                    __builtin_amdgcn_raw_ptr_buffer_load_lds(res0, dst, 16, off_a[i], so_x, 0, 0);
            }
        }
    };

#ifndef FM_B64
    constexpr int FRAG = 16;
#else
    constexpr int FRAG = 8;
#endif
    const int abase = (lrow & 7) * FM_AARR + (lrow >> 3) * 128 + FRAG * lh;
    int bbase[9];
#pragma unroll
    for (int r = 0; r < 3; ++r)
#pragma unroll
        for (int c = 0; c < 3; ++c) {
            const int n = (2 * pt + (lrow >> 4) + r) * 18 + (lrow & 15) + c;
            bbase[3 * r + c] = G::BOFF + (n & 7) * G::BARR + (n >> 3) * 128 + FRAG * lh;
        }

    f32x16 acc[9];
#pragma unroll
    for (int c = 0; c < 9; ++c)
#pragma unroll
        for (int r = 0; r < 16; ++r) acc[c][r] = 0.f;

#ifndef FM_PROBE
#define FM_PROBE 0
#endif
    auto compute = [&](int u) {
        const unsigned char *st = smem + u * G::STAGE;
#ifdef FM_STAGGER
        if (wave >= 4) __builtin_amdgcn_s_sleep(FM_STAGGER);
#endif
#ifndef FM_B64
#pragma unroll
        for (int gi = 0; gi < 4 / G::KS; ++gi) {
            const int kg = ks + G::KS * gi;
            f32x4 x[9];
#pragma unroll
            for (int c = 0; c < 9; ++c) x[c] = *(const f32x4 *)(st + bbase[c] + 32 * kg);
            f32x4 an = *(const f32x4 *)(st + abase + 32 * kg);
            f32x4 rw[3][3], xt[9];
#pragma unroll
            for (int c = 0; c < 3; ++c) {
                rw[0][c] = x[c] - x[3 + c];
                rw[1][c] = x[3 + c];
                rw[2][c] = x[6 + c] - x[3 + c];
            }
#pragma unroll
            for (int p = 0; p < 3; ++p) {
                xt[3 * p] = rw[p][0] - rw[p][1];
                xt[3 * p + 1] = rw[p][1];
                xt[3 * p + 2] = rw[p][2] - rw[p][1];
            }
#pragma unroll
            for (int c = 0; c < 9; ++c) {
                const f32x4 ac = an;
                if (c + 1 < 9) an = *(const f32x4 *)(st + abase + (c + 1) * 512 + 32 * kg);
#pragma unroll
                for (int j = 0; j < 4; ++j)
                    acc[c] = __builtin_amdgcn_mfma_f32_32x32x2f32(ac[j], xt[c][j], acc[c], 0, 0, 0);
            }
        }
#else
#pragma unroll
        for (int gi = 0; gi < 8 / G::KS; ++gi) {
            const int kg = ks + G::KS * gi;
            f32x2 a[9], x[9];
#pragma unroll
            for (int c = 0; c < 9; ++c) a[c] = *(const f32x2 *)(st + abase + ((FM_PROBE & 2) ? 0 : c) * 512 + 16 * kg);
#pragma unroll
            for (int c = 0; c < 9; ++c) x[c] = *(const f32x2 *)(st + bbase[(FM_PROBE & 2) ? 0 : c] + 16 * kg);
            f32x2 rw[3][3], xt[9];
#pragma unroll
            for (int c = 0; c < 3; ++c) {
                rw[0][c] = x[c] - x[3 + c];
                rw[1][c] = x[3 + c];
                rw[2][c] = x[6 + c] - x[3 + c];
            }
#pragma unroll
            for (int p = 0; p < 3; ++p) {
                xt[3 * p] = rw[p][0] - rw[p][1];
                xt[3 * p + 1] = rw[p][1];
                xt[3 * p + 2] = rw[p][2] - rw[p][1];
            }
#pragma unroll
            for (int c = 0; c < 9; ++c) {
                acc[c] = __builtin_amdgcn_mfma_f32_32x32x2f32(a[c][0], xt[c][0], acc[c], 0, 0, 0);
                acc[c] = __builtin_amdgcn_mfma_f32_32x32x2f32(a[c][1], xt[c][1], acc[c], 0, 0, 0);
            }
        }
#endif
    };

    issue(0, 0);
    for (int ch = 0; ch < nchunks; ++ch) {
        asm volatile("s_waitcnt vmcnt(0)" ::: "memory");
        if (!(FM_PROBE & 4) || ch == 0) __builtin_amdgcn_s_barrier();
        if (ch + 1 < nchunks && (!(FM_PROBE & 1) || ch == 0)) issue((ch + 1) & 1, ch + 1);
        compute(ch & 1);
    }

    const int ecq = lane & 7;
    f32x4 bias4 = {0.f, 0.f, 0.f, 0.f};
    if (P.bias) bias4 = *(const f32x4 *)(P.bias + co0 + 4 * ecq);
    __builtin_amdgcn_s_barrier();
#pragma unroll
    for (int f = 0; f < 4; ++f) {
        const int fa = f >> 1, fb = f & 1;
        const f32x16 t = (acc[3 * fa + fb] + acc[3 * fa + fb + 1]) + (acc[3 * fa + 3 + fb] + acc[3 * fa + 4 + fb]);
        unsigned char *xt_ = smem + (wave * 4 + f) * 4096;
#pragma unroll
        for (int g = 0; g < 4; ++g) {
            const f32x4 v = {t[4 * g], t[4 * g + 1], t[4 * g + 2], t[4 * g + 3]};
            *(f32x4 *)(xt_ + lrow * 128 + (((2 * g + lh) ^ (lrow & 7)) << 4)) = v;
        }
    }
    __builtin_amdgcn_s_barrier();
    const GDst &D = P.dst[0];
#pragma unroll
    for (int fi = 0; fi < 4 / G::KS; ++fi) {
        const int f = ks + G::KS * fi;
        const int fa = f >> 1, fb = f & 1;
#pragma unroll
        for (int it = 0; it < 4; ++it) {
            const int px = 8 * it + (lane >> 3);
            const int xo = px * 128 + ((ecq ^ (px & 7)) << 4);
            f32x4 v = *(const f32x4 *)(smem + (pt * 4 + f) * 4096 + xo);
#pragma unroll
            for (int k = 1; k < G::KS; ++k) v += *(const f32x4 *)(smem + ((pt + G::PT * k) * 4 + f) * 4096 + xo);
            const int yy = oy + 2 * pt + (px >> 4), xx = ox + (px & 15);
            const long long o = (long long)b * D.sb + (long long)yy * D.sy + (long long)xx * D.sx +
                                (long long)fa * D.ph_y + (long long)fb * D.ph_x + co0 + 4 * ecq;
            v += bias4;
            if (P.bias_cls) {
                const int Y = 2 * yy + fa, X = 2 * xx + fb;
                const int cls = 3 * (Y == 0 ? 1 : Y == P.out_H - 1 ? 2 : 0) + (X == 0 ? 1 : X == P.out_W - 1 ? 2 : 0);
                if (cls) v += *(const f32x4 *)(P.bias_cls + cls * P.N + co0 + 4 * ecq);
            }
            if (ZOUT) *(f32x4 *)(P.zout + o) = v;
#pragma unroll
            for (int e = 0; e < 4; ++e) v[e] = act_fwd(v[e], P.act);
            *(f32x4 *)(D.p + o) = v;
        }
    }
#endif
}

}

bool min9_shape_ok(int mfma, int nsrc, const int *C, const int *nhwc, int Cout, int H, int W)
{
    if (mfma != 0 || nsrc != 2) return false;
    for (int s = 0; s < 2; ++s)
        if (!nhwc[s] || (C[s] & 31)) return false;
    return (Cout & 31) == 0 && (W % 16) == 0 && (H % 4) == 0 && H >= 4;
}

int min9_prepare_fwd(const float *w, float *wt, int Cout, int Ctot, hipStream_t st)
{
    const size_t n = (size_t)Cout * Ctot;
    hipLaunchKernelGGL(min9_fwd_weights_kernel, dim3((unsigned)((n + 255) / 256)), dim3(256), 0, st, w, wt, Cout, Ctot);
    DVSOF_LAUNCH_CHECK();
    return DVSOF_OK;
}

template <int NR, bool ZOUT>
static int fm_launch(const GConvParams &P, int grid, hipStream_t st)
{
    typedef FMGeom<NR> G;
    static bool attr_set = false;
    if (!attr_set) {
        DVSOF_HIP_TRY(hipFuncSetAttribute((const void *)fwd_min_f32_kernel<NR, ZOUT>,
                                          hipFuncAttributeMaxDynamicSharedMemorySize, G::LDS));
        attr_set = true;
    }
    hipLaunchKernelGGL((fwd_min_f32_kernel<NR, ZOUT>), dim3(grid), dim3(FM_NT), G::LDS, st, P);
    DVSOF_LAUNCH_CHECK();
    conv_note_kernel(NR == 8 ? DVSOF_KERNEL_FWD_MIN8 : DVSOF_KERNEL_FWD_MIN4, 0);
    return DVSOF_OK;
}

int fwd_min_launch(const GConvParams &P, hipStream_t st)
{
    for (int s = 0; s < 2; ++s) {
        const GSrc &S = P.src[s];
        if (!S.p || (reinterpret_cast<uintptr_t>(S.p) & 15) || ((S.sb | S.sy | S.sx) & 3) || S.sc != 1) return DVSOF_EINVAL;
    }
    const GDst &D = P.dst[0];
    if (D.addend || D.addend2 || D.actsrc || D.sc != 1 || ((D.sb | D.sy | D.sx | D.ph_y | D.ph_x) & 3)) return DVSOF_EINVAL;
    if ((reinterpret_cast<uintptr_t>(D.p) & 15) || (reinterpret_cast<uintptr_t>(P.zout) & 15) ||
        (reinterpret_cast<uintptr_t>(P.W) & 15) || (reinterpret_cast<uintptr_t>(P.bias) & 15) ||
        (reinterpret_cast<uintptr_t>(P.bias_cls) & 15))
        return DVSOF_EINVAL;
    const long long per_row = (long long)P.B * (P.Wv / 16) * (P.N / 32);
    int nr = 4;
    if (P.Hv % 8 == 0 && per_row * (P.Hv / 8) >= 256) nr = 8;
    const int grid = (int)(per_row * (P.Hv / nr));
    const bool z = P.zout != nullptr;
    if (nr == 8) return z ? fm_launch<8, true>(P, grid, st) : fm_launch<8, false>(P, grid, st);
    return z ? fm_launch<4, true>(P, grid, st) : fm_launch<4, false>(P, grid, st);
}
```

Baseline: 3289 samples/s.

## Specialise min conv kernel epilogues and precompute grid division and patch offsets

Templates the fwd_min and dgrad_min MFMA kernels on the epilogue variant (relu, mish, class bias, head), so unused addend and activation branches are removed at compile time. Integer divisions for block decoding are replaced with host-precomputed magic multipliers, and the per-lane patch offsets and edge masks are hoisted out of the per-item setup. Accumulator zeroing is folded into the first MFMA, and the resident dgrad path is specialised to two chunks. The aim is to cut scalar and vector ALU overhead and register pressure, at the cost of more kernel instantiations and extra code complexity.

```diff
diff --git a/dvs_of_training_framework_amd/conv.py b/dvs_of_training_framework_amd/conv.py
--- a/dvs_of_training_framework_amd/conv.py
+++ b/dvs_of_training_framework_amd/conv.py
@@ -56,7 +56,11 @@
 
 def last_kernel(kind):
     v = _lib.lib().dvsof_conv2d_last_kernel(kind)
-    return v & 255, v >> 8
+    return v & 255, (v >> 8) & 255
+
+
+def last_kernel_variant(kind):
+    return _lib.lib().dvsof_conv2d_last_kernel(kind) >> 16
 
 
 def make_desc(srcs, B, H, W, Cout, ksize=3, stride=1, pad=1, upsample=False,
diff --git a/dvs_of_training_framework_amd/csrc/conv_api.hip b/dvs_of_training_framework_amd/csrc/conv_api.hip
--- a/dvs_of_training_framework_amd/csrc/conv_api.hip
+++ b/dvs_of_training_framework_amd/csrc/conv_api.hip
@@ -3,6 +3,7 @@
 static thread_local int t_last_kernel[3] = {0, 0, 0};
 static thread_local int t_kind = 0;
 void conv_note_kernel(int family, int mode) { t_last_kernel[t_kind] = family | mode << 8; }
+void conv_note_variant(int variant) { t_last_kernel[t_kind] = (t_last_kernel[t_kind] & 0xffff) | variant << 16; }
 static void conv_begin(int kind)
 {
     t_kind = kind;
diff --git a/dvs_of_training_framework_amd/csrc/conv_common.h b/dvs_of_training_framework_amd/csrc/conv_common.h
--- a/dvs_of_training_framework_amd/csrc/conv_common.h
+++ b/dvs_of_training_framework_amd/csrc/conv_common.h
@@ -101,6 +101,23 @@
     int coff, Cin_tot;
 };
 
+struct GridDiv {
+    unsigned d, m, one;
+};
+template <typename T = unsigned>
+__device__ __forceinline__ T grid_div(bool exact, T n, const GridDiv &g)
+{
+    return exact ? __umulhi(n, g.m) + (n & g.one) : n / g.d;
+}
+template <typename T = unsigned>
+inline bool grid_div_make(T d, long long nmax, GridDiv &g)
+{
+    g.d = d;
+    g.m = d < 2 ? 0u : (unsigned)(((1ull << 32) + d - 1) / d);
+    g.one = d < 2 ? ~0u : 0u;
+    return d >= 1 && nmax >= 0 && (unsigned long long)nmax * d < (1ull << 32);
+}
+
 __device__ __forceinline__ float mish_t(float x, float &n)
 {
     n = __builtin_amdgcn_exp2f(fminf(x, 20.f) * 1.4426950408889634f);
diff --git a/dvs_of_training_framework_amd/csrc/conv_host.h b/dvs_of_training_framework_amd/csrc/conv_host.h
--- a/dvs_of_training_framework_amd/csrc/conv_host.h
+++ b/dvs_of_training_framework_amd/csrc/conv_host.h
@@ -19,6 +19,7 @@
 ConvClass conv_classify(const dvsof_conv_desc_t *d);
 
 void conv_note_kernel(int family, int mode);
+void conv_note_variant(int variant);
 
 int gconv_launch(const GConvParams &P, int tile_hint, hipStream_t st);
 int gconv_pick_tile(long long m, long long n);
diff --git a/dvs_of_training_framework_amd/csrc/dgrad_min.hip b/dvs_of_training_framework_amd/csrc/dgrad_min.hip
--- a/dvs_of_training_framework_amd/csrc/dgrad_min.hip
+++ b/dvs_of_training_framework_amd/csrc/dgrad_min.hip
@@ -46,22 +46,30 @@
     }
 }
 
-template <int IPW>
-__global__ __launch_bounds__(DM_NT) void dgrad_min_f32_kernel(const GConvParams P, const int total)
+struct DMGrid {
+    GridDiv nct, nbx, nby;
+    int exact;
+};
+
+enum {
+    DM_EP_GENERIC = 0,
+    DM_EP_PLAIN = 1,
+    DM_EP_ACT = 2,
+    DM_EP_HEAD = 3
+};
+constexpr int dm_variant(int ep, int act) { return ep < DM_EP_ACT ? ep : 2 * ep + act - 3; }
+
+template <int IPW, int EP, int ACT>
+__global__ __launch_bounds__(DM_NT) void dgrad_min_f32_kernel(const GConvParams P, const int total, const DMGrid dv)
 {
 #if defined(__HIP_DEVICE_COMPILE__)
-    typedef float f32x2 __attribute__((ext_vector_type(2)));
     extern __shared__ __attribute__((aligned(1024))) unsigned char smem[];
     const int tid = threadIdx.x, lane = tid & 63;
     const int wave = __builtin_amdgcn_readfirstlane(tid >> 6);
     const int pt = wave & 3, ks = wave >> 2;
     const int lrow = lane & 31, lh = lane >> 5;
-    const int H = P.Ho, W = P.Wo;
-    const int FH = 2 * H, FW = 2 * W;
     const int Cout = P.Cin_tot, Ctot = P.N;
-    const int nbx = W / 16, nby = H / DM_NR;
-    const int nct = Ctot / 64;
-    const int nchunks = Cout / 16;
+    const int nct = (int)dv.nct.d;
 
     unsigned wg = blockIdx.x;
     {
@@ -69,8 +77,9 @@
         wg = x * q + min(x, r) + (wg >> 3);
     }
     constexpr bool RES = IPW == 0;
-    const int rows = RES ? (int)gridDim.x / nct : 1;
-    const int item0 = RES ? ((int)wg / nct) * nct + (int)wg % nct : (int)wg * IPW;
+    const int nchunks = RES ? 2 : Cout / 16;
+    const int rows = RES ? (int)grid_div(dv.exact, gridDim.x, dv.nct) : 1;
+    const int item0 = RES ? (int)wg : (int)wg * IPW;
     const int istep = RES ? rows * nct : 1;
     const int item1 = RES ? total : item0 + IPW;
 
@@ -79,42 +88,51 @@
     const __amdgpu_buffer_rsrc_t gres = __builtin_amdgcn_make_buffer_rsrc(
         (void *)(GS.p - ((long long)GS.sy + GS.sx)), 0, 0x7fffffff, 0x00020000);
 
+    static_assert(DM_AP >= 32 && DM_LPW - DM_AP / 8 <= 8, "edge bits of the patch rounds: one register");
+    unsigned offl[DM_LPW], ebits = 0;
+#pragma unroll
+    for (int i = 0; i < DM_LPW; ++i) {
+        const int p = wave + 8 * i;
+        offl[i] = DM_OOB;
+        if (p < DM_AP) {
+            const int m = p / 9, pp = p - 9 * m;
+            const int j = 16 * pp + (lane >> 2);
+            const int c = j >> 4, r = 4 * (j & 15) + m;
+            offl[i] = (((unsigned)c * (unsigned)Ctot + (unsigned)r) * (unsigned)Cout + 4u * (lane & 3)) * 4u;
+        } else if (p < DM_NPIECE) {
+            const int pb = p - DM_AP;
+            const int arr = pb / DM_BPA, pp = pb - DM_BPA * arr;
+            const int pr = 4 * (16 * pp + (lane >> 2)) + (arr & 3);
+            if (pr < DM_NPAIR) {
+                const int n = 2 * pr + (arr >> 2);
+                const int fr = n / 34, fc = n - 34 * fr;
+                offl[i] = (unsigned)((fr * GS.sy + fc * GS.sx + 4 * (lane & 3)) * 4);
+                const unsigned e = (fr == 0 ? 1u : 0u) | (fr == 2 * DM_NR + 1 ? 2u : 0u) | (fc == 0 ? 4u : 0u) |
+                                   (fc == 33 ? 8u : 0u);
+                if (i >= DM_AP / 8) ebits |= e << (4 * (i - DM_AP / 8));
+            }
+        }
+    }
     unsigned off[DM_LPW];
     int ci0 = 0, b = 0, oy = 0, ox = 0, wbase = 0, gbase = 0, blk_ = 0;
     auto setup = [&](int item) {
-        const int ct64 = item % nct, blk = item / nct;
-        blk_ = blk;
-        ci0 = 64 * ct64;
-        const int bx = blk % nbx, by = (blk / nbx) % nby;
-        b = blk / (nbx * nby);
-        oy = DM_NR * by;
-        ox = 16 * bx;
+        const unsigned blk = grid_div(dv.exact, (unsigned)item, dv.nct), ct64 = (unsigned)item - blk * dv.nct.d;
+        const unsigned t = grid_div(dv.exact, blk, dv.nbx), bx = blk - t * dv.nbx.d;
+        const unsigned bb_ = grid_div(dv.exact, t, dv.nby), by = t - bb_ * dv.nby.d;
+        blk_ = (int)blk;
+        ci0 = 64 * (int)ct64;
+        b = (int)bb_;
+        oy = DM_NR * (int)by;
+        ox = 16 * (int)bx;
         wbase = __builtin_amdgcn_readfirstlane((int)((size_t)ci0 * Cout * 4));
         gbase = __builtin_amdgcn_readfirstlane(
             (int)(((long long)b * GS.sb + (long long)(2 * oy) * GS.sy + (long long)(2 * ox) * GS.sx) * 4));
-#pragma unroll
-        for (int i = 0; i < DM_LPW; ++i) {
-            const int p = wave + 8 * i;
-            if (p < DM_AP) {
-                const int m = p / 9, pp = p - 9 * m;
-                const int j = 16 * pp + (lane >> 2);
-                const int c = j >> 4, r = 4 * (j & 15) + m;
-                off[i] = (unsigned)((((size_t)c * Ctot + r) * Cout + 4 * (lane & 3)) * 4);
-            } else if (p < DM_NPIECE) {
-                off[i] = DM_OOB;
-                const int pb = p - DM_AP;
-                const int arr = pb / DM_BPA, pp = pb - DM_BPA * arr;
-                const int pr = 4 * (16 * pp + (lane >> 2)) + (arr & 3);
-                if (pr < DM_NPAIR) {
-                    const int n = 2 * pr + (arr >> 2);
-                    const int fr = n / 34, fc = n - 34 * fr;
-                    if (((unsigned)(2 * oy + fr - 1) < (unsigned)FH) & ((unsigned)(2 * ox + fc - 1) < (unsigned)FW))
-                        off[i] = (unsigned)((fr * GS.sy + fc * GS.sx + 4 * (lane & 3)) * 4);
-                }
-            } else {
-                off[i] = DM_OOB;
-            }
-        }
+        const unsigned out = (by == 0 ? 1u : 0u) | (by == dv.nby.d - 1 ? 2u : 0u) | (bx == 0 ? 4u : 0u) |
+                             (bx == dv.nbx.d - 1 ? 8u : 0u);
+        const unsigned hit = ebits & (unsigned)__builtin_amdgcn_readfirstlane((int)(out * 0x11111111u));
+#pragma unroll
+        for (int i = 0; i < DM_LPW; ++i)
+            off[i] = (i >= DM_AP / 8 && (hit & (15u << (4 * (i - DM_AP / 8))))) ? DM_OOB : offl[i];
     };
 
     bool with_w = true;
@@ -122,16 +140,22 @@
         unsigned char *st = smem + stage_idx * DM_STAGE;
         const int so_w = __builtin_amdgcn_readfirstlane(wbase + ch * 64);
         const int so_g = __builtin_amdgcn_readfirstlane(gbase + ch * 64);
-#pragma unroll
-        for (int i = 0; i < DM_LPW; ++i) {
+        if (!RES || with_w) {
+#pragma unroll
+            for (int i = 0; i <= DM_AP / 8; ++i) {
+                const int p = wave + 8 * i;
+                if (p < DM_AP) {
+                    const int m = p / 9, pp = p - 9 * m;
+                    __attribute__((address_space(3))) void *dst =
+                        (__attribute__((address_space(3))) void *)(st + m * DM_AARR + pp * 1024);
+                    __builtin_amdgcn_raw_ptr_buffer_load_lds(wres, dst, 16, off[i], so_w, 0, 0);
+                }
+            }
+        }
+#pragma unroll
+        for (int i = DM_AP / 8; i < DM_LPW; ++i) {
             const int p = wave + 8 * i;
-            if (p < DM_AP) {
-                if (RES && !with_w) continue;
-                const int m = p / 9, pp = p - 9 * m;
-                __attribute__((address_space(3))) void *dst =
-                    (__attribute__((address_space(3))) void *)(st + m * DM_AARR + pp * 1024);
-                __builtin_amdgcn_raw_ptr_buffer_load_lds(wres, dst, 16, off[i], so_w, 0, 0);
-            } else if (p < DM_NPIECE) {
+            if (p >= DM_AP && p < DM_NPIECE) {
                 const int pb = p - DM_AP;
                 const int arr = pb / DM_BPA, pp = pb - DM_BPA * arr;
                 __attribute__((address_space(3))) void *dst =
@@ -142,6 +166,7 @@
     };
 
     const int abase = (lrow & 3) * DM_AARR + (lrow >> 2) * 64 + 16 * lh;
+    const int abase_t[2] = {abase + (8 * ks) * 64, abase + (8 * (1 - ks)) * 64};
     int bb[4][2];
     {
         const int li = lrow >> 4, lj = lrow & 15;
@@ -157,7 +182,7 @@
     f32x16 acc[2];
 
     typedef float f32x4_ __attribute__((ext_vector_type(4)));
-    auto compute = [&](int u_) {
+    auto compute = [&](int u_, bool first) {
         const unsigned char *st = smem + u_ * DM_STAGE;
         const int ko = 32 * ks;
         f32x4_ g[4][4];
@@ -183,11 +208,25 @@
         for (int t = 0; t < 2; ++t)
 #pragma unroll
             for (int c = 0; c < 9; ++c) {
-                const f32x4_ a = *(const f32x4_ *)(st + abase + (16 * c + 8 * t) * 64 + ko);
-#pragma unroll
-                for (int j = 0; j < 4; ++j)
-                    acc[t] = __builtin_amdgcn_mfma_f32_32x32x2f32(a[j], s[c][j], acc[t], 0, 0, 0);
-            }
+                const f32x4_ a = *(const f32x4_ *)(st + abase_t[t] + (16 * c) * 64 + ko);
+#pragma unroll
+                for (int j = 0; j < 4; ++j) {
+                    const f32x16 zero = {0.f, 0.f, 0.f, 0.f, 0.f, 0.f, 0.f, 0.f, 0.f, 0.f, 0.f, 0.f, 0.f, 0.f, 0.f, 0.f};
+                    acc[t] = __builtin_amdgcn_mfma_f32_32x32x2f32(a[j], s[c][j], first && c == 0 && j == 0 ? zero : acc[t],
+                                                                  0, 0, 0);
+                }
+            }
+    };
+    auto step = [&](int item, int ch, bool first) {
+        asm volatile("s_waitcnt vmcnt(0)" ::: "memory");
+        __builtin_amdgcn_s_barrier();
+        if (ch + 1 < nchunks) issue((ch + 1) & 1, ch + 1);
+        else if (item + istep < item1) {
+            with_w = false;
+            setup(item + istep);
+            issue((ch + 1) & 1, 0);
+        }
+        compute(ch & 1, first);
     };
 
     if (item0 >= item1) return;
@@ -196,59 +235,64 @@
 #pragma unroll
     for (int item = item0; item < item1; item += istep) {
         const int e_ci0 = ci0, e_b = b, e_oy = oy, e_ox = ox, e_blk = blk_;
-#pragma unroll
-        for (int t = 0; t < 2; ++t)
-#pragma unroll
-            for (int r = 0; r < 16; ++r) acc[t][r] = 0.f;
-        for (int ch = 0; ch < nchunks; ++ch) {
-            asm volatile("s_waitcnt vmcnt(0)" ::: "memory");
-            __builtin_amdgcn_s_barrier();
-            if (ch + 1 < nchunks) issue((ch + 1) & 1, ch + 1);
-            else if (item + istep < item1) {
-                with_w = false;
-                setup(item + istep);
-                issue((ch + 1) & 1, 0);
-            }
-            compute(ch & 1);
-        }
+        step(item, 0, true);
+        if (RES) step(item, 1, false);
+        else
+            for (int ch = 1; ch < nchunks; ++ch) step(item, ch, false);
 
         unsigned char *xch = RES ? smem + DM_STAGE + DM_BOFF : smem + ((nchunks - 1) & 1) * DM_STAGE;
+        typedef const __attribute__((address_space(4))) GConvParams *KArgs;
+        KArgs Pk = (KArgs)__builtin_amdgcn_kernarg_segment_ptr();
+        asm volatile("" : "+s"(Pk));
         const int cit = e_ci0 + 32 * ks;
-        const int c_first = P.dst[0].C;
+        const int c_first = Pk->dst[0].C;
         const int sel = cit >= c_first ? 1 : 0;
-        const GDst &D = P.dst[sel];
+        const auto &D = Pk->dst[sel];
         const int cm = cit - (sel ? c_first : 0);
+        constexpr bool GEN = EP == DM_EP_GENERIC;
+        const float *const actsrc = GEN || EP >= DM_EP_ACT ? D.actsrc : nullptr;
+        const bool f_add = GEN && D.addend, f_add2 = GEN && D.addend2;
+        const bool f_act = GEN ? actsrc != nullptr : EP >= DM_EP_ACT && sel == 0;
+        const bool f_head = GEN ? D.head_w != nullptr : EP == DM_EP_HEAD && sel == 0;
+        const bool f_part = GEN && D.head_part;
+        const int bwd_act = GEN ? Pk->bwd_act : ACT;
         int le = lane;
         asm volatile("" : "+v"(le));
         const int ecq = le & 7, elrow = le & 31, elh = le >> 5;
+        const long long ebase = (long long)e_b * D.sb + (long long)(e_oy + 2 * pt) * D.sy + (long long)e_ox * D.sx + cm;
+        unsigned eo[4];
+#pragma unroll
+        for (int it = 0; it < 4; ++it)
+            eo[it] = (unsigned)((it >> 1) * D.sy + (8 * (it & 1) + (le >> 3)) * D.sx + 4 * ecq) * 4u;
+        auto at = [&](const float *q, int it) { return (const f32x4 *)((const char *)(q + ebase) + eo[it]); };
         f32x4 hw0 = {0.f, 0.f, 0.f, 0.f}, hw1 = hw0;
-        if (D.head_w) {
+        f32x4 ead[4], ead2[4], eas[4], ehx[4];
+        float eg0[4], eg1[4];
+        const bool hx_own = f_part && D.head_x != actsrc;
+        if (f_head) {
             hw0 = *(const f32x4 *)(D.head_w + cm + 4 * ecq);
             hw1 = *(const f32x4 *)(D.head_w + D.C + cm + 4 * ecq);
-        }
-        long long eo[4];
-        f32x4 ead[4], ead2[4], eas[4], ehx[4];
-        float eg0[4], eg1[4];
-        const bool hx_own = D.head_part && D.head_x != D.actsrc;
+            const int Wl = Pk->Wo;
+            const long long hwp = (long long)Pk->Ho * Wl;
+            const float *g0 = D.head_g + (((long long)e_b * 2) * hwp + (long long)(e_oy + 2 * pt) * Wl + e_ox);
+#pragma unroll
+            for (int it = 0; it < 4; ++it) {
+                const unsigned r = (unsigned)((it >> 1) * Wl + 8 * (it & 1) + (le >> 3));
+                eg0[it] = g0[r];
+                eg1[it] = (g0 + hwp)[r];
+            }
+        }
 #pragma unroll
         for (int it = 0; it < 4; ++it) {
-            const int px = 8 * it + (le >> 3);
-            const int yy = e_oy + 2 * pt + (px >> 4), xx = e_ox + (px & 15);
-            eo[it] = (long long)e_b * D.sb + (long long)yy * D.sy + (long long)xx * D.sx + cm + 4 * ecq;
-            if (D.addend) ead[it] = *(const f32x4 *)(D.addend + eo[it]);
-            if (D.addend2) ead2[it] = *(const f32x4 *)(D.addend2 + eo[it]);
-            if (D.actsrc) eas[it] = *(const f32x4 *)(D.actsrc + eo[it]);
-            if (hx_own) ehx[it] = *(const f32x4 *)(D.head_x + eo[it]);
-            if (D.head_w) {
-                const long long hwp = (long long)H * W, r = (long long)yy * W + xx;
-                eg0[it] = D.head_g[((long long)e_b * 2) * hwp + r];
-                eg1[it] = D.head_g[((long long)e_b * 2 + 1) * hwp + r];
-            }
+            if (f_add) ead[it] = *at(D.addend, it);
+            if (f_add2) ead2[it] = *at(D.addend2, it);
+            if (f_act) eas[it] = *at(actsrc, it);
+            if (hx_own) ehx[it] = *at(D.head_x, it);
         }
         __builtin_amdgcn_s_barrier();
-        f32x16 mine = ks ? acc[1] : acc[0];
+        f32x16 mine = acc[0];
         {
-            const f32x16 other = ks ? acc[0] : acc[1];
+            const f32x16 other = acc[1];
             unsigned char *r1 = xch + wave * 4096;
 #pragma unroll
             for (int g = 0; g < 4; ++g)
@@ -278,23 +322,23 @@
             const int px = 8 * it + (le >> 3);
             const int xo = px * 128 + ((ecq ^ (px & 7)) << 4);
             f32x4 v = *(const f32x4 *)(r2 + xo);
-            if (D.addend) v += ead[it];
-            if (D.addend2) v += ead2[it];
-            if (D.head_w) v += eg0[it] * hw0 + eg1[it] * hw1;
-            if (D.head_part) {
+            if (f_add) v += ead[it];
+            if (f_add2) v += ead2[it];
+            if (f_head) v += eg0[it] * hw0 + eg1[it] * hw1;
+            if (f_part) {
                 const f32x4 xv = hx_own ? ehx[it] : eas[it];
                 ha0 += eg0[it] * xv;
                 ha1 += eg1[it] * xv;
                 hs0 += eg0[it];
                 hs1 += eg1[it];
             }
-            if (D.actsrc) {
-#pragma unroll
-                for (int e = 0; e < 4; ++e) v[e] *= act_bwd(eas[it][e], P.bwd_act);
-            }
-            *(f32x4 *)(D.p + eo[it]) = v;
-        }
-        if (D.head_part) {
+            if (f_act) {
+#pragma unroll
+                for (int e = 0; e < 4; ++e) v[e] *= act_bwd(eas[it][e], bwd_act);
+            }
+            *(f32x4 *)((char *)(D.p + ebase) + eo[it]) = v;
+        }
+        if (f_part) {
 #pragma unroll
             for (int o_ = 8; o_ < 64; o_ <<= 1) {
 #pragma unroll
@@ -345,6 +389,43 @@
     hipLaunchKernelGGL(min9_dgrad_weights_kernel, grid, dim3(256), 0, st, w, wq, Cout, Ctot);
     DVSOF_LAUNCH_CHECK();
     return DVSOF_OK;
+}
+
+namespace {
+
+int dm_epilogue(const GConvParams &P, int &act)
+{
+    const GDst &D0 = P.dst[0], &D1 = P.dst[1];
+    if (D1.addend || D1.addend2 || D1.actsrc || D1.head_w || D1.head_part) return DM_EP_GENERIC;
+    if (D0.addend || D0.addend2 || D0.head_part) return DM_EP_GENERIC;
+    if (!D0.actsrc) return D0.head_w ? DM_EP_GENERIC : DM_EP_PLAIN;
+    if (P.bwd_act != ACT_RELU && P.bwd_act != ACT_MISH) return DM_EP_GENERIC;
+    act = P.bwd_act;
+    return D0.head_w ? DM_EP_HEAD : DM_EP_ACT;
+}
+
+template <int IPW, int EP, int ACT>
+int dm_launch(const GConvParams &P, unsigned grid, int total, const DMGrid &dv, hipStream_t st)
+{
+    static bool attr_set = false;
+    if (!attr_set) {
+        DVSOF_HIP_TRY(hipFuncSetAttribute((const void *)dgrad_min_f32_kernel<IPW, EP, ACT>,
+                                          hipFuncAttributeMaxDynamicSharedMemorySize, DM_LDS));
+        attr_set = true;
+    }
+    hipLaunchKernelGGL((dgrad_min_f32_kernel<IPW, EP, ACT>), dim3(grid), dim3(DM_NT), DM_LDS, st, P, total, dv);
+    DVSOF_LAUNCH_CHECK();
+    conv_note_kernel(IPW == 0 ? DVSOF_KERNEL_DGRAD_MIN0 : DVSOF_KERNEL_DGRAD_MIN1, 0);
+    conv_note_variant(dm_variant(EP, ACT));
+    return DVSOF_OK;
+}
+
+template <int EP, int ACT>
+int dm_launch_res(bool res, const GConvParams &P, int total, const DMGrid &dv, hipStream_t st)
+{
+    return res ? dm_launch<0, EP, ACT>(P, 256u, total, dv, st) : dm_launch<1, EP, ACT>(P, (unsigned)total, total, dv, st);
+}
+
 }
 
 int dgrad_min_launch(const GConvParams &P, hipStream_t st)
@@ -360,29 +441,23 @@
              reinterpret_cast<uintptr_t>(D.head_w)) & 15)
             return DVSOF_EINVAL;
     }
-    static bool attr_set = false;
-    if (!attr_set) {
-        DVSOF_HIP_TRY(hipFuncSetAttribute((const void *)dgrad_min_f32_kernel<1>,
-                                          hipFuncAttributeMaxDynamicSharedMemorySize, DM_LDS));
-        attr_set = true;
-    }
     const long long total = (long long)P.B * (P.Ho / DM_NR) * (P.Wo / 16) * (P.N / 64);
     const int nchunks = P.Cin_tot / 16;
-    const int nct = P.N / 64;
-    if (nchunks == 2 && 256 % nct == 0 && total >= 2 * 256) {
-        static bool attr0 = false;
-        if (!attr0) {
-            DVSOF_HIP_TRY(hipFuncSetAttribute((const void *)dgrad_min_f32_kernel<0>,
-                                              hipFuncAttributeMaxDynamicSharedMemorySize, DM_LDS));
-            attr0 = true;
-        }
-        hipLaunchKernelGGL(dgrad_min_f32_kernel<0>, dim3(256), dim3(DM_NT), DM_LDS, st, P, (int)total);
-        DVSOF_LAUNCH_CHECK();
-        conv_note_kernel(DVSOF_KERNEL_DGRAD_MIN0, 0);
-        return DVSOF_OK;
-    }
-    hipLaunchKernelGGL(dgrad_min_f32_kernel<1>, dim3((unsigned)total), dim3(DM_NT), DM_LDS, st, P, (int)total);
-    DVSOF_LAUNCH_CHECK();
-    conv_note_kernel(DVSOF_KERNEL_DGRAD_MIN1, 0);
-    return DVSOF_OK;
-}
+    if (total <= 0 || total > 0x7fffffff) return DVSOF_EINVAL;
+    DMGrid dv;
+    const bool e0 = grid_div_make((unsigned)(P.N / 64), total, dv.nct);
+    const bool e1 = grid_div_make((unsigned)(P.Wo / 16), total, dv.nbx);
+    const bool e2 = grid_div_make((unsigned)(P.Ho / DM_NR), total, dv.nby);
+    dv.exact = e0 && e1 && e2;
+    int act = ACT_RELU;
+    const int ep = dm_epilogue(P, act);
+    const bool res = nchunks == 2 && 256 % (int)dv.nct.d == 0 && total >= 2 * 256;
+    int rc;
+    if (ep == DM_EP_PLAIN) rc = dm_launch_res<DM_EP_PLAIN, ACT_NONE>(res, P, (int)total, dv, st);
+    else if (ep == DM_EP_ACT && act == ACT_RELU) rc = dm_launch_res<DM_EP_ACT, ACT_RELU>(res, P, (int)total, dv, st);
+    else if (ep == DM_EP_ACT) rc = dm_launch_res<DM_EP_ACT, ACT_MISH>(res, P, (int)total, dv, st);
+    else if (ep == DM_EP_HEAD && act == ACT_RELU) rc = dm_launch_res<DM_EP_HEAD, ACT_RELU>(res, P, (int)total, dv, st);
+    else if (ep == DM_EP_HEAD) rc = dm_launch_res<DM_EP_HEAD, ACT_MISH>(res, P, (int)total, dv, st);
+    else rc = dm_launch_res<DM_EP_GENERIC, ACT_NONE>(res, P, (int)total, dv, st);
+    return rc;
+}
diff --git a/dvs_of_training_framework_amd/csrc/fwd_min.hip b/dvs_of_training_framework_amd/csrc/fwd_min.hip
--- a/dvs_of_training_framework_amd/csrc/fwd_min.hip
+++ b/dvs_of_training_framework_amd/csrc/fwd_min.hip
@@ -48,30 +48,44 @@
     }
 }
 
-template <int NR, bool ZOUT>
-__global__ __launch_bounds__(FM_NT) void fwd_min_f32_kernel(const GConvParams P)
+struct FMGrid {
+    GridDiv nco, nbx, nby;
+    int exact;
+};
+
+enum {
+    FM_EP_GENERIC = 0,
+    FM_EP_RELU = 1,
+    FM_EP_RELU_CLS = 2,
+    FM_EP_MISH = 3,
+    FM_EP_MISH_CLS = 4
+};
+
+template <int NR, int EP>
+__global__ __launch_bounds__(FM_NT) void fwd_min_f32_kernel(const GConvParams P, const FMGrid dv)
 {
 #if defined(__HIP_DEVICE_COMPILE__)
     typedef FMGeom<NR> G;
+#ifdef FM_B64
     typedef float f32x2 __attribute__((ext_vector_type(2)));
+#endif
     extern __shared__ __attribute__((aligned(1024))) unsigned char smem[];
     const int tid = threadIdx.x, lane = tid & 63;
     const int wave = __builtin_amdgcn_readfirstlane(tid >> 6);
     const int pt = wave % G::PT, ks = wave / G::PT;
     const int lrow = lane & 31, lh = lane >> 5;
     const int H = P.Hv, W = P.Wv;
-    const int nbx = W / 16, nby = H / NR;
 
     unsigned wg = blockIdx.x;
     {
         const unsigned total = gridDim.x, x = wg & 7u, q = total >> 3, r = total & 7u;
         wg = x * q + min(x, r) + (wg >> 3);
     }
-    const int nco = P.N / 32;
-    const int cot = (int)(wg % (unsigned)nco), blk = (int)(wg / (unsigned)nco);
-    const int co0 = 32 * cot;
-    const int bx = blk % nbx, by = (blk / nbx) % nby, b = blk / (nbx * nby);
-    const int oy = NR * by, ox = 16 * bx;
+    const unsigned blk = grid_div(dv.exact, wg, dv.nco), cot = wg - blk * dv.nco.d;
+    const unsigned t_ = grid_div(dv.exact, blk, dv.nbx), bx = blk - t_ * dv.nbx.d;
+    const unsigned b_ = grid_div(dv.exact, t_, dv.nby), by = t_ - b_ * dv.nby.d;
+    const int co0 = 32 * (int)cot, b = (int)b_;
+    const int oy = NR * (int)by, ox = 16 * (int)bx;
 
     const GSrc &S0 = P.src[0], &S1 = P.src[1];
     unsigned off_a[G::LPW], off_b[G::LPW - FM_APA];
@@ -86,7 +100,7 @@
             if (j < 36) {
                 const int R = 8 * j + m;
                 const int c = R >> 5, r = R & 31;
-                off_a[i] = (unsigned)((((size_t)c * P.N + co0 + r) * P.Cin_tot + 4 * (lane & 7)) * 4);
+                off_a[i] = (((unsigned)c * (unsigned)P.N + (unsigned)(co0 + r)) * (unsigned)P.Cin_tot + 4u * (lane & 7)) * 4u;
             }
         } else {
             const int pb = p - FM_AP;
@@ -153,16 +167,20 @@
             bbase[3 * r + c] = G::BOFF + (n & 7) * G::BARR + (n >> 3) * 128 + FRAG * lh;
         }
 
+    constexpr bool PEEL = NR == 4;
     f32x16 acc[9];
-#pragma unroll
-    for (int c = 0; c < 9; ++c)
-#pragma unroll
-        for (int r = 0; r < 16; ++r) acc[c][r] = 0.f;
+    if (!PEEL) {
+#pragma unroll
+        for (int c = 0; c < 9; ++c)
+#pragma unroll
+            for (int r = 0; r < 16; ++r) acc[c][r] = 0.f;
+    }
 
 #ifndef FM_PROBE
 #define FM_PROBE 0
 #endif
-    auto compute = [&](int u) {
+    auto compute = [&](int u, bool first) {
+        const f32x16 zero = {0.f, 0.f, 0.f, 0.f, 0.f, 0.f, 0.f, 0.f, 0.f, 0.f, 0.f, 0.f, 0.f, 0.f, 0.f, 0.f};
         const unsigned char *st = smem + u * G::STAGE;
 #ifdef FM_STAGGER
         if (wave >= 4) __builtin_amdgcn_s_sleep(FM_STAGGER);
@@ -194,7 +212,8 @@
                 if (c + 1 < 9) an = *(const f32x4 *)(st + abase + (c + 1) * 512 + 32 * kg);
 #pragma unroll
                 for (int j = 0; j < 4; ++j)
-                    acc[c] = __builtin_amdgcn_mfma_f32_32x32x2f32(ac[j], xt[c][j], acc[c], 0, 0, 0);
+                    acc[c] = __builtin_amdgcn_mfma_f32_32x32x2f32(ac[j], xt[c][j], first && gi == 0 && j == 0 ? zero : acc[c],
+                                                                  0, 0, 0);
             }
         }
 #else
@@ -221,24 +240,39 @@
             }
 #pragma unroll
             for (int c = 0; c < 9; ++c) {
-                acc[c] = __builtin_amdgcn_mfma_f32_32x32x2f32(a[c][0], xt[c][0], acc[c], 0, 0, 0);
+                acc[c] = __builtin_amdgcn_mfma_f32_32x32x2f32(a[c][0], xt[c][0], first && gi == 0 ? zero : acc[c], 0, 0, 0);
                 acc[c] = __builtin_amdgcn_mfma_f32_32x32x2f32(a[c][1], xt[c][1], acc[c], 0, 0, 0);
             }
         }
 #endif
     };
 
-    issue(0, 0);
-    for (int ch = 0; ch < nchunks; ++ch) {
+    auto step = [&](int ch, bool first) {
         asm volatile("s_waitcnt vmcnt(0)" ::: "memory");
         if (!(FM_PROBE & 4) || ch == 0) __builtin_amdgcn_s_barrier();
         if (ch + 1 < nchunks && (!(FM_PROBE & 1) || ch == 0)) issue((ch + 1) & 1, ch + 1);
-        compute(ch & 1);
-    }
-
-    const int ecq = lane & 7;
+        compute(ch & 1, first);
+    };
+    issue(0, 0);
+    if (PEEL) {
+        step(0, true);
+        for (int ch = 1; ch < nchunks; ++ch) step(ch, false);
+    } else {
+        int ch = 0;
+        do step(ch, false);
+        while (++ch < nchunks);
+    }
+
+    constexpr bool GEN = EP == FM_EP_GENERIC;
+    const bool f_bias = GEN ? P.bias != nullptr : true;
+    const bool f_cls = GEN ? P.bias_cls != nullptr : EP == FM_EP_RELU_CLS || EP == FM_EP_MISH_CLS;
+    const bool f_zout = GEN ? P.zout != nullptr : EP >= FM_EP_MISH;
+    const int act = GEN ? P.act : EP >= FM_EP_MISH ? ACT_MISH : ACT_RELU;
+    int le = lane;
+    asm volatile("" : "+v"(le));
+    const int ecq = le & 7;
     f32x4 bias4 = {0.f, 0.f, 0.f, 0.f};
-    if (P.bias) bias4 = *(const f32x4 *)(P.bias + co0 + 4 * ecq);
+    if (f_bias) bias4 = *(const f32x4 *)(P.bias + co0 + 4 * ecq);
     __builtin_amdgcn_s_barrier();
 #pragma unroll
     for (int f = 0; f < 4; ++f) {
@@ -253,30 +287,35 @@
     }
     __builtin_amdgcn_s_barrier();
     const GDst &D = P.dst[0];
+    const int y0 = oy + 2 * pt;
+    const long long obase = (long long)b * D.sb + (long long)y0 * D.sy + (long long)ox * D.sx + co0;
+    unsigned eo[4];
+#pragma unroll
+    for (int it = 0; it < 4; ++it) eo[it] = (unsigned)((it >> 1) * D.sy + (8 * (it & 1) + (le >> 3)) * D.sx + 4 * ecq) * 4u;
+    const bool edge = f_cls && (oy == 0 || 2 * (oy + NR) >= P.out_H || ox == 0 || 2 * (ox + 16) >= P.out_W);
 #pragma unroll
     for (int fi = 0; fi < 4 / G::KS; ++fi) {
         const int f = ks + G::KS * fi;
         const int fa = f >> 1, fb = f & 1;
+        const long long pbase = obase + (long long)fa * D.ph_y + (long long)fb * D.ph_x;
 #pragma unroll
         for (int it = 0; it < 4; ++it) {
-            const int px = 8 * it + (lane >> 3);
+            const int px = 8 * it + (le >> 3);
             const int xo = px * 128 + ((ecq ^ (px & 7)) << 4);
             f32x4 v = *(const f32x4 *)(smem + (pt * 4 + f) * 4096 + xo);
 #pragma unroll
             for (int k = 1; k < G::KS; ++k) v += *(const f32x4 *)(smem + ((pt + G::PT * k) * 4 + f) * 4096 + xo);
-            const int yy = oy + 2 * pt + (px >> 4), xx = ox + (px & 15);
-            const long long o = (long long)b * D.sb + (long long)yy * D.sy + (long long)xx * D.sx +
-                                (long long)fa * D.ph_y + (long long)fb * D.ph_x + co0 + 4 * ecq;
             v += bias4;
-            if (P.bias_cls) {
+            if (edge) {
+                const int yy = y0 + (px >> 4), xx = ox + (px & 15);
                 const int Y = 2 * yy + fa, X = 2 * xx + fb;
                 const int cls = 3 * (Y == 0 ? 1 : Y == P.out_H - 1 ? 2 : 0) + (X == 0 ? 1 : X == P.out_W - 1 ? 2 : 0);
                 if (cls) v += *(const f32x4 *)(P.bias_cls + cls * P.N + co0 + 4 * ecq);
             }
-            if (ZOUT) *(f32x4 *)(P.zout + o) = v;
-#pragma unroll
-            for (int e = 0; e < 4; ++e) v[e] = act_fwd(v[e], P.act);
-            *(f32x4 *)(D.p + o) = v;
+            if (f_zout) *(f32x4 *)((char *)(P.zout + pbase) + eo[it]) = v;
+#pragma unroll
+            for (int e = 0; e < 4; ++e) v[e] = act_fwd(v[e], act);
+            *(f32x4 *)((char *)(D.p + pbase) + eo[it]) = v;
         }
     }
 #endif
@@ -300,20 +339,35 @@
     return DVSOF_OK;
 }
 
-template <int NR, bool ZOUT>
-static int fm_launch(const GConvParams &P, int grid, hipStream_t st)
+template <int NR, int EP>
+static int fm_launch(const GConvParams &P, int grid, const FMGrid &dv, hipStream_t st)
 {
     typedef FMGeom<NR> G;
     static bool attr_set = false;
     if (!attr_set) {
-        DVSOF_HIP_TRY(hipFuncSetAttribute((const void *)fwd_min_f32_kernel<NR, ZOUT>,
+        DVSOF_HIP_TRY(hipFuncSetAttribute((const void *)fwd_min_f32_kernel<NR, EP>,
                                           hipFuncAttributeMaxDynamicSharedMemorySize, G::LDS));
         attr_set = true;
     }
-    hipLaunchKernelGGL((fwd_min_f32_kernel<NR, ZOUT>), dim3(grid), dim3(FM_NT), G::LDS, st, P);
+    hipLaunchKernelGGL((fwd_min_f32_kernel<NR, EP>), dim3(grid), dim3(FM_NT), G::LDS, st, P, dv);
     DVSOF_LAUNCH_CHECK();
     conv_note_kernel(NR == 8 ? DVSOF_KERNEL_FWD_MIN8 : DVSOF_KERNEL_FWD_MIN4, 0);
+    conv_note_variant(EP);
     return DVSOF_OK;
+}
+
+template <int EP>
+static int fm_launch_nr(int nr, const GConvParams &P, int grid, const FMGrid &dv, hipStream_t st)
+{
+    return nr == 8 ? fm_launch<8, EP>(P, grid, dv, st) : fm_launch<4, EP>(P, grid, dv, st);
+}
+
+static int fm_epilogue(const GConvParams &P)
+{
+    if (!P.bias) return FM_EP_GENERIC;
+    if (P.act == ACT_RELU && !P.zout) return P.bias_cls ? FM_EP_RELU_CLS : FM_EP_RELU;
+    if (P.act == ACT_MISH && P.zout) return P.bias_cls ? FM_EP_MISH_CLS : FM_EP_MISH;
+    return FM_EP_GENERIC;
 }
 
 int fwd_min_launch(const GConvParams &P, hipStream_t st)
@@ -331,8 +385,19 @@
     const long long per_row = (long long)P.B * (P.Wv / 16) * (P.N / 32);
     int nr = 4;
     if (P.Hv % 8 == 0 && per_row * (P.Hv / 8) >= 256) nr = 8;
-    const int grid = (int)(per_row * (P.Hv / nr));
-    const bool z = P.zout != nullptr;
-    if (nr == 8) return z ? fm_launch<8, true>(P, grid, st) : fm_launch<8, false>(P, grid, st);
-    return z ? fm_launch<4, true>(P, grid, st) : fm_launch<4, false>(P, grid, st);
-}
+    const long long total = per_row * (P.Hv / nr);
+    if (total <= 0 || total > 0x7fffffff) return DVSOF_EINVAL;
+    const int grid = (int)total;
+    FMGrid dv;
+    const bool e0 = grid_div_make((unsigned)(P.N / 32), total, dv.nco);
+    const bool e1 = grid_div_make((unsigned)(P.Wv / 16), total, dv.nbx);
+    const bool e2 = grid_div_make((unsigned)(P.Hv / nr), total, dv.nby);
+    dv.exact = e0 && e1 && e2;
+    switch (fm_epilogue(P)) {
+    case FM_EP_RELU: return fm_launch_nr<FM_EP_RELU>(nr, P, grid, dv, st);
+    case FM_EP_RELU_CLS: return fm_launch_nr<FM_EP_RELU_CLS>(nr, P, grid, dv, st);
+    case FM_EP_MISH: return fm_launch_nr<FM_EP_MISH>(nr, P, grid, dv, st);
+    case FM_EP_MISH_CLS: return fm_launch_nr<FM_EP_MISH_CLS>(nr, P, grid, dv, st);
+    default: return fm_launch_nr<FM_EP_GENERIC>(nr, P, grid, dv, st);
+    }
+}
```

Result: no change. 3320 samples/s (median of 6 runs) (+1.0%).
